# Eun0/XMC-GAN

Hardware: AMD Instinct MI355X
Metric: images/sec per G+D step (higher is better)
Workload: dtype bf16; 1 GPU; 256x256 COCO-shaped synthetic batch, 256 images per GPU, one full G+D iteration (D step + G step + Adam x2), df_gan_damsm_nomagp.yml; per_gpu_batch=256, global_batch=256, image_size=256, cfg=df_gan_damsm_nomagp.yml, parallelism=dp1, hipgraph=True, losses_finite=True, workload_name=headline

## Files before the change

include/xmc_gan_hip.h:

```cpp
#ifndef XMC_GAN_HIP_H
#define XMC_GAN_HIP_H

#include <stdint.h>

#ifdef __cplusplus
extern "C" {
#endif

#define XMC_ABI_VERSION 12

enum { XMC_BF16 = 0, XMC_F32 = 1 };
enum { XMC_HALF_IS_BF16 = 0, XMC_HALF_IS_F16 = 1 };
enum { XMC_ACT_NONE = 0, XMC_ACT_LRELU = 1, XMC_ACT_TANH = 2, XMC_ACT_RELU = 3 };
enum { XMC_EINVAL = -1, XMC_EALIGN = -2, XMC_ESHAPE = -3 };

#define XMC_MAX_TAPS 16
#define XMC_MAX_CLASSES 4

typedef struct XmcConvDesc {
    const void* src;
    const void* wpk;
    void* dst;
    const float* bias;
    const void* res;
    const float* alpha_dev;
    int32_t N, SH, SW, CS;
    int32_t DH, DW, CD;
    int32_t MH, MW;
    int32_t SA, DA;
    int32_t src_shift;
    int32_t ntaps, nclass;
    int32_t CDw;
    int32_t act;
    int32_t dtype;
    int32_t out_dtype;
    int8_t dh[XMC_MAX_CLASSES][XMC_MAX_TAPS];
    int8_t dw[XMC_MAX_CLASSES][XMC_MAX_TAPS];
    int8_t wi[XMC_MAX_CLASSES][XMC_MAX_TAPS];
    int8_t dph[XMC_MAX_CLASSES];
    int8_t dpw[XMC_MAX_CLASSES];
    const void* mask;
    float res_scale;
    int32_t res_mode;
    void* dst2;
    void* dst_pool;
    int32_t round_act;
    int32_t groups;
    int32_t post_act;
    float pool_scale;
    void* sign_bits;
    float* dot;
    const void* mask_bits;
    const void* sc_img;
    const void* sc_frag;
    const float* sc_bias;
    void* splitk_ws;
    int64_t splitk_ws_bytes;
    const void* wpk_lo;
} XmcConvDesc;

int xmc_abi_version(void);
int xmc_half_format(void);
const char* xmc_last_kernel(void);
int xmc_set_fixed_order(int on);
int xmc_set_prezeroed(int on);

int64_t xmc_conv_splitk_ws_bytes(const XmcConvDesc* d);

int xmc_conv_igemm(const XmcConvDesc* d, void* stream);

int xmc_conv_wgrad(const XmcConvDesc* d , float* dwp, void* stream);
#define XMC_BIAS_REPLICAS 16
int xmc_conv_wgrad_bias(const XmcConvDesc* d, float* dwp, float* dbias, void* stream);

int xmc_pack_weight(const float* w, void* wpk, int Co, int Ci, int KH, int KW, int rows_pad, int cols_pad,
                    int transpose , int dtype, const int32_t* row_perm , void* stream);
int xmc_pack_weight_grouped(const float* w, void* wpk, int Co, int Ci, int KH, int KW, int rows_pad, int cols_pad, int transpose,
                            int dtype, const int32_t* row_perm, int groups, void* stream);
int xmc_unpack_wgrad_grouped(const float* dwp, float* gw, int Co, int Ci, int KH, int KW, int rows_pad, int cols_pad,
                             const float* scale_dev, const int32_t* row_perm, int accumulate, int groups, void* stream);
#define XMC_PACK_MULTI_MAX 48
typedef struct XmcPackJob {
    const float* w;
    void* wpk;
    const int32_t* row_perm;
    int32_t Co, Ci, KHW, rows_pad, cols_pad, transpose, dtype, groups, upconv;
    int32_t lo;
} XmcPackJob;
int xmc_pack_weight_multi(const XmcPackJob* jobs , int njobs, void* stream);
int xmc_pack_weight_upconv(const float* w, void* wpk, int Co, int Ci, int rows_pad, int cols_pad, int transpose, int dtype,
                           void* stream);
int xmc_unpack_wgrad(const float* dwp, float* gw, int Co, int Ci, int KH, int KW, int rows_pad, int cols_pad,
                     const float* scale_dev, const int32_t* row_perm, int accumulate, void* stream);
int xmc_unpack_wgrad_bias(const float* dwp, float* gw, int Co, int Ci, int KH, int KW, int rows_pad, int cols_pad,
                          const float* scale_dev, const int32_t* row_perm, int accumulate,
                          const float* gb_replicas, float* gb, int CD, void* stream);
int xmc_unpack_wgrad_bias_dot(const float* dwp, float* gw, int Co, int Ci, int KH, int KW, int rows_pad, int cols_pad,
                              const float* scale_dev, const int32_t* row_perm, int accumulate,
                              const float* gb_replicas, float* gb, int CD, const float* bias_dot, float* dot, void* stream);

int xmc_nchw_to_nhwc8(const float* src , void* dst , int N, int C, int H, int W,
                      int dtype, void* stream);
int xmc_nhwc8_to_nchw(const void* src , float* dst , int N, int C, int H, int W,
                      int dtype, void* stream);

int xmc_lrelu(const void* x, void* y, int64_t n, float slope, int dtype, void* stream);
int xmc_lrelu_mask(const void* dy, const void* ref, void* dx, int64_t n, float slope, int dtype, void* stream);
int xmc_tanh(const void* x, void* y, int64_t n, int dtype, void* stream);
int xmc_signmask_apply(const void* dy, const void* bits, void* dx, int64_t n, float slope, int dtype, void* stream);
int xmc_conv_pw1x1_masked_src(const XmcConvDesc* d, const void* src_bits, void* src_masked, float slope, void* stream);
int xmc_conv_pw1x1_split(const XmcConvDesc* d, void* stream);
int xmc_conv_ptile_bits(const XmcConvDesc* d, void* stream);
int xmc_conv_ptile_scimg(const XmcConvDesc* d, void* stream);
int xmc_conv_wgrad_bits(const XmcConvDesc* d, float* dwp, void* stream);
int xmc_gtail_bwd(const XmcConvDesc* d, const void* img, float* dwp, float* dbias, int dw_rows, int grid_cap, void* stream);
int xmc_gentry_fwd(const void* x, const float* g0, const float* b0, const float* g1, const float* b1, const void* wpk, const float* bias,
                   void* h, void* sc, int N, int H, int W, int Cin, int Cout, int wrows, float slope, int dtype, int grid_cap, void* stream);
int xmc_gentry_bwd(const void* x, const void* dy, const void* dsc, const float* g0, const float* b0, const float* g1, const float* b1,
                   const void* wpk_t, void* dx, void* dx_pool, float* dg0, float* db0, float* dg1, float* db1, int N, int H, int W,
                   int Cin, int Cout, int wrows, float slope, int dtype, int grid_cap, void* stream);
int xmc_tanh_bwd(const void* dy, const void* y, void* dx, int64_t n, int dtype, void* stream);
int xmc_axpby(const void* a, const void* b, const float* alpha_dev, void* y, int64_t n, int dtype, void* stream);
int xmc_axpby_up(const void* a, const void* b, const float* alpha_dev, void* y, int N, int H, int W, int C, int dtype, void* stream);
int xmc_axpby_up_lrelu(const void* a, const void* b, const float* alpha_dev, void* y, int N, int H, int W, int C, int dtype, void* stream);
int xmc_scale(const void* x, const float* alpha_dev, void* y, int64_t n, int dtype, void* stream);
int xmc_dot(const void* a, const void* b, float* out, int64_t n, int dtype, void* stream);
enum { XMC_GP_BIAS = 1, XMC_GP_RELU = 2, XMC_GP_MASK = 4, XMC_GP_ATOMIC = 8 };
typedef struct XmcGemmProblem {
    const float* A;
    const float* B;
    const float* bias;
    const float* mask;
    float* C;
    float* rowsum;
    int32_t M, N, K;
    int32_t sa_i, sa_r, sb_j, sb_r;
    int32_t flags;
    int32_t tile0;
    int32_t reserved;
} XmcGemmProblem;
int xmc_gemm_group(const XmcGemmProblem* problems, int nproblems, void* stream);
int xmc_embedding_gather(const int64_t* ids, const float* table, float* out, int64_t n_tokens, int dim, int64_t vocab, void* stream);
int xmc_gru_bidir(const float* xproj, const float* w_hh, const float* b_hn, const int32_t* lens, float* words, float* sent, int B, int T,
                  int H, void* stream);
int xmc_lstm_bidir(const float* xproj, const float* w_hh, const int32_t* lens, float* words, float* sent, int B, int T, int H,
                   void* stream);
int xmc_roberta_embed_ln(const int64_t* ids, const int32_t* lens, const float* word, const float* pos, const float* type0,
                         const float* gamma, const float* beta, float* out, void* out16, int B, int T, int H, int64_t vocab, int npos,
                         int pad_idx, float eps, void* stream);
int xmc_add_layernorm(const float* x, const float* bias, const float* res, const float* gamma, const float* beta, float* out, void* out16,
                      int64_t rows, int H, float eps, void* stream);
int xmc_attention_short(const float* qkv, const int32_t* lens, void* out, int B, int T, int heads, int head_dim, int out_dtype,
                        void* stream);
int xmc_bias_gelu(const float* x, const float* bias, void* out, int64_t rows, int F, int out_dtype, void* stream);
int xmc_sbert_pool(const float* hidden, const int32_t* lens, float* words, float* sent, uint8_t* mask, int B, int T, int H, int L,
                   int normalize, void* stream);
int xmc_spectral_sigma(const float* W, float* u, float* v, float* scratch, float* sig, float* w_eff, int R, int C, int training,
                       float eps, void* stream);
int xmc_spectral_bwd(const float* g, const float* W, const float* u, const float* v, const float* sig, float* dot, float* dW,
                     int R, int C, void* stream);
int xmc_scale_mask_dot(const void* dy, const void* ref, const float* alpha_dev, void* g, float* dot, int64_t n, int dtype, void* stream);
int xmc_axpby_bwd(const void* dy, const void* b, const float* alpha_dev, void* db, void* da, float* dot,
                  int N, int H, int W, int C, int up, const void* ymask , int dtype, void* stream);
int xmc_colsum(const void* x, float* out, int64_t rows, int C, int dtype, void* stream);
int xmc_avgpool2(const void* x, void* y, int N, int H, int W, int C, int dtype, void* stream);
int xmc_upsample2(const void* x, void* y, int N, int H, int W, int C, float scale, int dtype, void* stream);
int xmc_sumpool2(const void* x, void* y, int N, int H, int W, int C, float scale, int dtype, void* stream);
int xmc_global_avgpool(const void* x, void* y, int N, int HW, int C, int dtype, int out_dtype, void* stream);
int xmc_global_avgpool_bwd(const void* dy, void* dx, int N, int HW, int C, int dtype, int in_dtype, void* stream);

int xmc_affine2_lrelu_fwd(const void* x, const float* g0, const float* b0, const float* g1, const float* b1,
                          void* y, int N, int HW, int C, int dtype, void* stream);
int xmc_affine2_lrelu_bwd(const void* x, const void* dy, const float* g0, const float* b0, const float* g1,
                          const float* b1, void* dx, float* dg0, float* db0, float* dg1, float* db1,
                          int N, int HW, int C, int dtype, void* stream);

int xmc_affine2_act_fwd(const void* x, const float* g0, const float* b0, const float* g1, const float* b1,
                        void* y, int N, int HW, int C, float slope, int dtype, void* stream);
int xmc_affine2_act_bwd(const void* x, const void* dy, const float* g0, const float* b0, const float* g1,
                        const float* b1, void* dx, float* dg0, float* db0, float* dg1, float* db1,
                        int N, int HW, int C, float slope, int dtype, void* stream);
int xmc_affine2_act_bwd_acc(const void* x, const void* dy, const float* g0, const float* b0, const float* g1,
                            const float* b1, void* dx, float* dg0, float* db0, float* dg1, float* db1, const void* dx_in,
                            int N, int HW, int C, float slope, int dtype, void* stream);
int xmc_affine2_act_bwd_dot(const void* x, const void* dy, const float* g0, const float* b0, const float* g1,
                            const float* b1, void* dx, float* dg0, float* db0, float* dg1, float* db1, const void* dx_in,
                            const float* alpha_dev, float* dot, int N, int HW, int C, float slope, int dtype, void* stream);
int xmc_affine2_act_bwd_dot_pool(const void* x, const void* dy, const float* g0, const float* b0, const float* g1,
                                 const float* b1, void* dx, float* dg0, float* db0, float* dg1, float* db1, const void* dx_in,
                                 const float* alpha_dev, float* dot, void* dx_pool, int N, int H, int W, int C, float slope,
                                 int dtype, void* stream);

int xmc_groupnorm_fwd(const void* x, const float* w, const float* b, void* y, float* stats, float* ws,
                      int N, int HW, int C, int G, float eps, float slope, int dtype, void* stream);
int xmc_groupnorm_bwd(const void* x, const void* dy, const float* w, const float* b, const float* stats, void* dx,
                      float* dw, float* db, float* ws, int N, int HW, int C, int G, float slope, int dtype, void* stream);
int64_t xmc_attn_pool_ws_floats(int N, int HW);
int xmc_attn_pool_fwd(const void* key, const float* q, const void* x, float* stats, float* ctx, float* ws, int N, int HW,
                      int ncon, int pk, int px, float scale, int dtype, void* stream);
int xmc_attn_pool_bwd(const void* key, const float* q, const void* x, const float* stats, const float* ctx, const float* dctx,
                      float* dq, void* dkey, void* dx, int N, int HW, int ncon, int pk, int px, float scale, int dtype, void* stream);
int xmc_attn_pool_bwd_acc(const void* key, const float* q, const void* x, const float* stats, const float* ctx, const float* dctx,
                          float* dq, void* dkey, void* dx, const void* dx_in, int N, int HW, int ncon, int pk, int px, float scale,
                          int dtype, void* stream);

int xmc_gvec_fwd(const float* xs, const float* xg, const float* W, const float* bias, float* y, int B, int G, int O, int Is, int Ig, void* stream);
int xmc_gvec_bwd(const float* xs, const float* xg, const float* W, const float* dy, float* dxs, float* dxg, float* dW, float* dbias,
                 int B, int G, int O, int Is, int Ig, void* stream);
int xmc_reasoner_fwd(const float* x, const float* We, const float* bn_w, const float* bn_b, float* run_mean, float* run_var, int training,
                     float momentum, float eps, float* y, float* pre, float* stat, int B, void* stream);
int xmc_reasoner_bwd(const float* x, const float* We, const float* bn_w, const float* bn_b, const float* pre, const float* stat, int batch_stats,
                     const float* dy, float* dx, float* dWe, float* dbn_w, float* dbn_b, int B, void* stream);
int xmc_word_ctx_fwd(const float* st, const float* w, const unsigned char* pad, float* ctx, float* prob, int B, int T, void* stream);
int xmc_word_ctx_bwd(const float* st, const float* w, const float* prob, const float* dctx, float* dst, float* dw, int B, int T, void* stream);
int xmc_word_keys_fwd(const float* kraw, const float* gnw, const float* gnb, float eps, float* kh, float* stat, int B, int T, void* stream);
int xmc_word_keys_bwd(const float* kraw, const float* gnw, const float* gnb, const float* stat, const float* dkh, float* dkraw, float* dgnw,
                      float* dgnb, int B, int T, void* stream);
int xmc_word_pool_fwd(const void* qmap, const float* kh, const unsigned char* pad, float* ctx, int N, int HW, int ncon, int pk, int T,
                      int dtype, void* stream);
int xmc_word_pool_bwd(const void* qmap, const float* kh, const unsigned char* pad, const float* dctx, void* dq, float* dkh, int N, int HW,
                      int ncon, int pk, int T, int dtype, void* stream);

int64_t xmc_contrastive_ws_bytes(int n, int D);
int xmc_contrastive_fwd(const float* A, const float* B, const float* labels, const float* inv_num_pos,
                        int n, int D, float* loss, void* ws, void* stream);
int xmc_contrastive_bwd(const float* A, const float* B, const float* labels, const float* inv_num_pos,
                        int n, int D, const float* dloss_dev, void* ws, float* dA, float* dB, void* stream);

int xmc_cosine_scores(const float* A, const float* B, int n, int D, float* S, void* ws, void* stream);

int xmc_hinge_fwd(const void* x, int stride, float sign, float* out, int64_t n, int dtype, void* stream);
int xmc_hinge_bwd(const void* x, int stride, float sign, const float* dloss_dev, void* dx, int64_t n, int dtype,
                  void* stream);

int xmc_cast(const void* x, void* y, int64_t n, int src_dtype, int dst_dtype, void* stream);

typedef struct XmcAdamEntry {
    float* param;
    const float* grad;
    float* m;
    float* v;
    int32_t* step;
    int64_t n;
} XmcAdamEntry;
int xmc_adam_chunk_elems(void);
int xmc_adam_step(const XmcAdamEntry* table_dev, int ntensors, const int32_t* chunks_dev, int nchunks,
                  float lr, float beta1, float beta2, float eps, float grad_scale, void* stream);
enum { XMC_ADAM_CHECK = 1, XMC_ADAM_UPDATE = 2, XMC_ADAM_RESCALE = 4 };
int xmc_adam_step_scaled(const XmcAdamEntry* table_dev, int ntensors, const int32_t* chunks_dev, int nchunks,
                         float lr, float beta1, float beta2, float eps, float* scale_dev, int32_t* flags_dev,
                         int mode, float growth, float backoff, int interval, void* stream);

typedef struct XmcEmaEntry {
    float* shadow;
    const float* param;
    int64_t n;
} XmcEmaEntry;
int xmc_ema_step(const XmcEmaEntry* table_dev, int ntensors, const int32_t* chunks_dev, int nchunks, float decay, int start,
                 int32_t* num_updates_dev, const int32_t* skip_flag_dev, int bump, void* stream);
int xmc_adam_ema_step(const XmcAdamEntry* table_dev, const XmcEmaEntry* ema_table_dev, int ntensors, const int32_t* chunks_dev,
                      int nchunks, float lr, float beta1, float beta2, float eps, float grad_scale, float decay, int start,
                      int32_t* num_updates_dev, int bump, void* stream);
int xmc_adam_ema_step_scaled(const XmcAdamEntry* table_dev, const XmcEmaEntry* ema_table_dev, int ntensors,
                             const int32_t* chunks_dev, int nchunks, float lr, float beta1, float beta2, float eps,
                             float* scale_dev, int32_t* flags_dev, int mode, float growth, float backoff, int interval,
                             float decay, int start, int32_t* num_updates_dev, int bump, void* stream);

int xmc_rows_sumsq(const float* x, float* ss, int B, int64_t cols, void* stream);
int xmc_gp_finish(const float* ss, int B, float* gp, float* coef, float inv_s2, void* stream);
int xmc_rows_scale(const float* x, const float* coef, const float* g, float* y, int B, int64_t cols, void* stream);

int xmc_concept_query_fwd(const float* sent, const float* Wq, const float* gnw, const float* gnb, float* q, float* qraw,
                          int B, int E, float eps, void* stream);
int xmc_concept_query_bwd(const float* sent, const float* Wq, const float* gnw, const float* qraw, const float* dq, float* dsent,
                          float* dWq, float* dgnw, float* dgnb, float* scratch, int B, int E, float eps, void* stream);
int xmc_concept_query_fwd_multi(const float* sent, const float* const* Wq, const float* const* gnw, const float* const* gnb, int S, float* q,
                                float* qraw, int B, int E, float eps, void* stream);
int xmc_concept_query_bwd_multi(const float* sent, const float* const* Wq, const float* const* gnw, int S, const float* qraw, const float* dq,
                                float* dsent, float* dWq, float* dgn, float* scratch, int B, int E, float eps, void* stream);
int xmc_concept_gquery_fwd(const float* q0, const float* Wq, const float* gnw, const float* gnb, float* q, float* qraw, int B,
                           float eps, void* stream);
int xmc_concept_gquery_bwd(const float* q0, const float* Wq, const float* gnw, const float* qraw, const float* dq, float* dq0,
                           float* dWq, float* dgnw, float* dgnb, int B, float eps, void* stream);
int xmc_concept_head_fwd(const float* ctx, const float* sent, const float* const* params, float* gamma, float* beta, float* hid,
                         int B, int E, void* stream);
int xmc_concept_head_fwd_pre(const float* ctx, const float* sent, const float* const* params, const float* a_pre, float* gamma, float* beta,
                             float* hid, int B, int E, void* stream);
int xmc_concept_head_bwd(const float* ctx, const float* sent, const float* hid, const float* const* params, const float* dgamma,
                         const float* dbeta, float* dctx, float* dsent, float* const* grads, float* scratch, int B, int E,
                         void* stream);
int xmc_concept_head_bwd_pre(const float* ctx, const float* sent, const float* hid, const float* const* params, const float* dgamma,
                             const float* dbeta, float* dctx, float* dsent, float* const* grads, float* scratch, int B, int E, void* stream);
int xmc_concept_outer_multi(const float* D, const float* X, const float* const* W, float* const* dW, int nW, int Rp, float* dX, int B, int C,
                            int ldw, void* stream);

int xmc_dstem_compose(const float* wi, const float* bi, const float* w0, const float* ws, const float* bs, float* W, float* bias, float* D,
                      float* DB, void* stream);
int xmc_dstem_compose_bwd(const float* wi, const float* bi, const float* w0, const float* ws, const float* dW, const float* dbias,
                          const float* dD, const float* dDB, float* dwi, float* dbi, float* dw0, float* dws, float* dbs, void* stream);
int xmc_dstem_pack(const float* wsets, void* wfrag, void* stream);
int xmc_dstem_pack_sc(const float* wsets, void* sc_frag, void* stream);
int xmc_dstem_fwd(const void* img, const void* wfrag, const float* bias, void* h1, void* sc, int N, int H, int W, float slope, void* stream);
int xmc_dstem_wgrad(const void* img, const void* dh1, const void* dsc, float* dw, float* dbias, int N, int H, int W, int skip_border,
                    void* stream);
int xmc_dstem_border_fwd(const void* img, const float* w, const float* bias, const float* D, const float* DB, void* frag_scratch ,
                         void* h1, int N, int H, int W, float slope, void* stream);
int xmc_dstem_border_wgrad(const void* img, const void* dh1, float* dD, float* dDB, int N, int H, int W, void* stream);
int xmc_dstem_dgrad(const void* dh1, const void* dsc, const float* wsets, const float* D, void* frag_scratch, void* dimg, int N, int H, int W,
                    void* stream);

#define XMC_DIFFAUG_PARTS 64
int xmc_diffaug_sums(const void* x, const float* params, float* parts, int N, int H, int W, int C, int cut, int transposed, int dtype,
                     void* stream);
int xmc_diffaug_apply(const void* x, const float* params, const float* parts, void* y, int N, int H, int W, int C, int cut, int transposed,
                      int linear_only, int dtype, void* stream);

int xmc_image_to_u8(const void* x, uint8_t* y, int N, int H, int W, int dtype, void* stream);
int xmc_image_minmax(const void* x, float* parts, int N, int H, int W, int dtype, void* stream);
int xmc_image_grid_u8(const void* x, const float* parts, uint8_t* grid, int N, int H, int W, int nrow, int padding, int dtype, void* stream);

int xmc_fid_resize_u8(const uint8_t* src, float* dst, int N, int H, int W, int OH, int OW, void* stream);
#define XMC_POOL_MAX 0
#define XMC_POOL_AVG_VALID 1
#define XMC_POOL_AVG_PAD 2
int xmc_pool3x3(const float* x, float* y, int N, int H, int W, int C, int mode, int stride, void* stream);
int xmc_resize_bilinear_f32(const float* src, float* dst, int N, int H, int W, int OH, int OW, void* stream);
int xmc_fid_moments(const float* x, double* sum, double* outer, int B, int D, void* stream);

int xmc_rprecision(const float* img, const float* txt, const int32_t* cand, int32_t* rank, float* score, int N, int M, int K, int D, void* stream);

int xmc_crop_flip_normalize(const uint8_t* pool, int64_t pool_bytes, const int64_t* offsets, const int32_t* hw, int N, const int32_t* params,
                            const float* table, float* out, int B, int S, void* stream);

int xmc_caption_gather(const float* sent_tab, const float* tok_tab, int64_t tok_rows, const int64_t* tok_offsets, const int32_t* lens, int N,
                       const int32_t* rows, int B, int E, int T, float* words, float* sent, uint8_t* mask, void* stream);

int xmc_manifold_slices(int Nq, int Nc, int slices);
int xmc_row_sqnorm(const float* x, float* n2, int N, int D, void* stream);
int xmc_knn_radius2(const float* x, const float* n2, float* r2, float* ws, int64_t ws_bytes, int N, int D, int k, int slices, void* stream);
int xmc_manifold_count(const float* a, const float* na2, const float* b, const float* nb2, const float* rb2, int32_t* count, float* near2,
                       void* ws, int64_t ws_bytes, int Na, int Nb, int D, int slices, void* stream);

int xmc_poly_mmd_tiles(int m);
int xmc_poly_mmd_sums(const float* real, const float* fake, const int32_t* idx_real, const int32_t* idx_fake, double* out, double* ws,
                      int64_t ws_bytes, int Nr, int Nf, int D, int S, int m, void* stream);
int64_t xmc_inception_score_ws_bytes(int N, int C, int splits);
int xmc_inception_score(const float* logits, int64_t ld, double* H, double* P, double* ws, int64_t ws_bytes, int N, int C, int splits,
                        void* stream);

#ifdef __cplusplus
}
#endif
#endif
```

xmc-gan_amd/csrc/adam.hip:

```cpp
#include "common.h"

namespace {
constexpr int NT = 256;
constexpr int CHUNK = NT * 4 * 4;

__global__ void adam_check_kernel(const XmcAdamEntry* __restrict__ tab, const int2* __restrict__ chunks, int* __restrict__ si) {
    const int2 c = chunks[blockIdx.x];
    const XmcAdamEntry e = tab[c.x];
    const int64_t base = (int64_t)c.y * CHUNK;
    const int64_t lim = e.n - base < CHUNK ? e.n - base : CHUNK;
    const float* g = e.grad + base;
    bool bad = false;
    if ((e.n & 3) == 0) {
        for (int i = threadIdx.x * 4; i < lim; i += NT * 4) {
            const f32x4 G = *reinterpret_cast<const f32x4*>(g + i);
            bad |= !(fabsf(G[0]) < INFINITY) | !(fabsf(G[1]) < INFINITY) | !(fabsf(G[2]) < INFINITY) | !(fabsf(G[3]) < INFINITY);
        }
    } else {
        for (int i = threadIdx.x; i < lim; i += NT) bad |= !(fabsf(g[i]) < INFINITY);
    }
    if (__builtin_amdgcn_ballot_w64(bad) != 0 && (threadIdx.x & 63) == 0) atomicOr(si, 1);
}
__global__ void scaler_update_kernel(float* __restrict__ sf, int* __restrict__ si, float growth, float backoff, int interval) {
    if (threadIdx.x != 0 || blockIdx.x != 0) return;
    float sc = sf[0];
    const int bad = si[0];
    if (bad) {
        sc = fmaxf(sc * backoff, 1.f);
        si[1] = 0;
        si[3] += 1;
    } else if (++si[1] >= interval) {
        sc = fminf(sc * growth, 16777216.f);
        si[1] = 0;
    }
    sf[0] = sc;
    sf[1] = 1.f / sc;
    si[2] = bad;
    si[0] = 0;
}

__global__ void adam_kernel(const XmcAdamEntry* __restrict__ tab, const int2* __restrict__ chunks,
                            float lr, float b1, float b2, float eps, float gs, const float* __restrict__ sf,
                            const int* __restrict__ si) {
    if (si && *si) return;
    if (sf) gs *= sf[1];
    const int2 c = chunks[blockIdx.x];
    const XmcAdamEntry e = tab[c.x];
    const int t = *e.step + 1;
    const float bc1 = 1.f - powf(b1, (float)t), bc2s = sqrtf(1.f - powf(b2, (float)t));
    const float step_size = lr / bc1;
    const int64_t base = (int64_t)c.y * CHUNK;
    const int64_t lim = e.n - base < CHUNK ? e.n - base : CHUNK;
    float* p = e.param + base; const float* g = e.grad + base; float* m = e.m + base; float* v = e.v + base;
    if ((e.n & 3) == 0) {
        for (int i = threadIdx.x * 4; i < lim; i += NT * 4) {
            f32x4 P = *reinterpret_cast<f32x4*>(p + i), G = *reinterpret_cast<const f32x4*>(g + i) * gs;
            f32x4 M = *reinterpret_cast<f32x4*>(m + i), V = *reinterpret_cast<f32x4*>(v + i);
#pragma unroll
            for (int k = 0; k < 4; ++k) {
                M[k] = b1 * M[k] + (1.f - b1) * G[k];
                V[k] = b2 * V[k] + (1.f - b2) * G[k] * G[k];
                P[k] -= step_size * M[k] / (sqrtf(V[k]) / bc2s + eps);
            }
            *reinterpret_cast<f32x4*>(p + i) = P; *reinterpret_cast<f32x4*>(m + i) = M; *reinterpret_cast<f32x4*>(v + i) = V;
        }
    } else {
        for (int i = threadIdx.x; i < lim; i += NT) {
            float G = g[i] * gs;
            float M = b1 * m[i] + (1.f - b1) * G;
            float V = b2 * v[i] + (1.f - b2) * G * G;
            p[i] -= step_size * M / (sqrtf(V) / bc2s + eps);
            m[i] = M; v[i] = V;
        }
    }
}
__global__ void adam_bump_kernel(const XmcAdamEntry* tab, int n, const int* __restrict__ si) {
    if (si && *si) return;
    int i = blockIdx.x * blockDim.x + threadIdx.x;
    if (i < n) *tab[i].step += 1;
}
}

extern "C" int xmc_adam_chunk_elems(void) { return CHUNK; }

extern "C" int xmc_adam_step(const XmcAdamEntry* table_dev, int ntensors, const int32_t* chunks_dev, int nchunks,
                             float lr, float beta1, float beta2, float eps, float grad_scale, void* stream) {
    if (!table_dev || !chunks_dev || ntensors < 1 || nchunks < 1) return XMC_EINVAL;
    hipStream_t st = reinterpret_cast<hipStream_t>(stream);
    hipLaunchKernelGGL(adam_kernel, dim3(nchunks), dim3(NT), 0, st, table_dev, reinterpret_cast<const int2*>(chunks_dev), lr, beta1, beta2, eps,
                       grad_scale, (const float*)nullptr, (const int*)nullptr);
    hipLaunchKernelGGL(adam_bump_kernel, dim3((ntensors + NT - 1) / NT), dim3(NT), 0, st, table_dev, ntensors, (const int*)nullptr);
    XMC_LAUNCH_CHECK();
    return 0;
}

extern "C" int xmc_adam_step_scaled(const XmcAdamEntry* table_dev, int ntensors, const int32_t* chunks_dev, int nchunks,
                                    float lr, float beta1, float beta2, float eps, float* scale_dev, int32_t* flags_dev,
                                    int mode, float growth, float backoff, int interval, void* stream) {
    if (!table_dev || !chunks_dev || ntensors < 1 || nchunks < 1 || !scale_dev || !flags_dev || interval < 1 || (mode & 7) == 0) return XMC_EINVAL;
    hipStream_t st = reinterpret_cast<hipStream_t>(stream);
    const int2* ch = reinterpret_cast<const int2*>(chunks_dev);
    if (mode & XMC_ADAM_CHECK) hipLaunchKernelGGL(adam_check_kernel, dim3(nchunks), dim3(NT), 0, st, table_dev, ch, flags_dev);
    if (mode & XMC_ADAM_UPDATE) {
        hipLaunchKernelGGL(adam_kernel, dim3(nchunks), dim3(NT), 0, st, table_dev, ch, lr, beta1, beta2, eps, 1.f, (const float*)scale_dev,
                           (const int*)flags_dev);
        hipLaunchKernelGGL(adam_bump_kernel, dim3((ntensors + NT - 1) / NT), dim3(NT), 0, st, table_dev, ntensors, (const int*)flags_dev);
    }
    if (mode & XMC_ADAM_RESCALE) hipLaunchKernelGGL(scaler_update_kernel, dim3(1), dim3(64), 0, st, scale_dev, flags_dev, growth, backoff, interval);
    XMC_LAUNCH_CHECK();
    return 0;
}

namespace {
__device__ __forceinline__ bool aligned16(const void* a) { return (reinterpret_cast<uintptr_t>(a) & 15) == 0; }
__device__ __forceinline__ float ema_elem(float e, float p, float w, bool copy) { return copy ? p : __builtin_fmaf(w, p - e, e); }

__global__ void ema_kernel(const XmcEmaEntry* __restrict__ tab, const int2* __restrict__ chunks, float decay, int start,
                           const int* __restrict__ nupd, const int* __restrict__ si) {
    if (si && *si) return;
    const int2 c = chunks[blockIdx.x];
    const XmcEmaEntry t = tab[c.x];
    const bool copy = *nupd < start;
    const float w = 1.f - decay;
    const int64_t base = (int64_t)c.y * CHUNK;
    const int lim = (int)(t.n - base < CHUNK ? t.n - base : CHUNK);
    float* e = t.shadow + base; const float* p = t.param + base;
    int body = 0;
    if (aligned16(e) && aligned16(p)) {
        body = lim & ~3;
        for (int i = threadIdx.x * 4; i < body; i += NT * 4) {
            f32x4 E = *reinterpret_cast<f32x4*>(e + i);
            const f32x4 P = *reinterpret_cast<const f32x4*>(p + i);
#pragma unroll
            for (int k = 0; k < 4; ++k) E[k] = ema_elem(E[k], P[k], w, copy);
            *reinterpret_cast<f32x4*>(e + i) = E;
        }
    }
    for (int i = body + threadIdx.x; i < lim; i += NT) e[i] = ema_elem(e[i], p[i], w, copy);
}

template <bool FMA>
__device__ __forceinline__ float adam_elem(float P, float G, float& M, float& V, float b1, float b2, float step_size, float bc2s,
                                           float eps) {
#pragma clang fp contract(off)
    const float t = (1.f - b1) * G, u = ((1.f - b2) * G) * G;
    M = FMA ? __builtin_fmaf(b1, M, t) : b1 * M + t;
    V = FMA ? __builtin_fmaf(b2, V, u) : b2 * V + u;
    return P - (step_size * M) / (sqrtf(V) / bc2s + eps);
}

template <bool FMA>
__device__ __forceinline__ void adam_ema_chunk(float* p, const float* g, float* m, float* v, float* sh, int lim, float gs, float b1,
                                               float b2, float step_size, float bc2s, float eps, float w, bool copy) {
    int body = 0;
    if (aligned16(p) && aligned16(g) && aligned16(m) && aligned16(v) && aligned16(sh)) {
        body = lim & ~3;
        for (int i = threadIdx.x * 4; i < body; i += NT * 4) {
            f32x4 P = *reinterpret_cast<f32x4*>(p + i), G = *reinterpret_cast<const f32x4*>(g + i);
            f32x4 M = *reinterpret_cast<f32x4*>(m + i), V = *reinterpret_cast<f32x4*>(v + i);
#pragma unroll
            for (int k = 0; k < 4; ++k) {
                float Mk = M[k], Vk = V[k];
                P[k] = adam_elem<FMA>(P[k], G[k] * gs, Mk, Vk, b1, b2, step_size, bc2s, eps);
                M[k] = Mk; V[k] = Vk;
            }
            *reinterpret_cast<f32x4*>(p + i) = P; *reinterpret_cast<f32x4*>(m + i) = M; *reinterpret_cast<f32x4*>(v + i) = V;
            if (sh) {
                f32x4 E = *reinterpret_cast<f32x4*>(sh + i);
#pragma unroll
                for (int k = 0; k < 4; ++k) E[k] = ema_elem(E[k], P[k], w, copy);
                *reinterpret_cast<f32x4*>(sh + i) = E;
            }
        }
    }
    for (int i = body + threadIdx.x; i < lim; i += NT) {
        float M = m[i], V = v[i];
        const float P = adam_elem<FMA>(p[i], g[i] * gs, M, V, b1, b2, step_size, bc2s, eps);
        p[i] = P; m[i] = M; v[i] = V;
        if (sh) sh[i] = ema_elem(sh[i], P, w, copy);
    }
}

__global__ void adam_ema_kernel(const XmcAdamEntry* __restrict__ tab, const XmcEmaEntry* __restrict__ ema,
                                const int2* __restrict__ chunks, float lr, float b1, float b2, float eps, float gs,
                                const float* __restrict__ sf, const int* __restrict__ si, float decay, int start,
                                const int* __restrict__ nupd) {
    if (si && *si) return;
    if (sf) gs *= sf[1];
    const int2 c = chunks[blockIdx.x];
    const XmcAdamEntry t = tab[c.x];
    const int step = *t.step + 1;
    const float bc1 = 1.f - powf(b1, (float)step), bc2s = sqrtf(1.f - powf(b2, (float)step));
    const float step_size = lr / bc1;
    const bool copy = *nupd < start;
    const float w = 1.f - decay;
    const int64_t base = (int64_t)c.y * CHUNK;
    const int lim = (int)(t.n - base < CHUNK ? t.n - base : CHUNK);
    float* sh = ema[c.x].shadow;
    if (sh) sh += base;
    if ((t.n & 3) == 0) adam_ema_chunk<true>(t.param + base, t.grad + base, t.m + base, t.v + base, sh, lim, gs, b1, b2, step_size, bc2s, eps, w, copy);
    else adam_ema_chunk<false>(t.param + base, t.grad + base, t.m + base, t.v + base, sh, lim, gs, b1, b2, step_size, bc2s, eps, w, copy);
}

__global__ void ema_bump_kernel(const XmcAdamEntry* tab, int n, const int* __restrict__ si, int* nupd, int bump) {
    if (si && *si) return;
    const int i = blockIdx.x * blockDim.x + threadIdx.x;
    if (tab && i < n) *tab[i].step += 1;
    if (bump && i == 0) *nupd += 1;
}

bool ema_args_ok(float decay, int start, const int32_t* nupd) { return nupd && decay >= 0.f && decay < 1.f && start >= 0; }
}

extern "C" int xmc_ema_step(const XmcEmaEntry* table_dev, int ntensors, const int32_t* chunks_dev, int nchunks, float decay,
                            int start, int32_t* num_updates_dev, const int32_t* skip_flag_dev, int bump, void* stream) {
    if (!table_dev || !chunks_dev || ntensors < 1 || nchunks < 1 || !ema_args_ok(decay, start, num_updates_dev)) return XMC_EINVAL;
    hipStream_t st = reinterpret_cast<hipStream_t>(stream);
    hipLaunchKernelGGL(ema_kernel, dim3(nchunks), dim3(NT), 0, st, table_dev, reinterpret_cast<const int2*>(chunks_dev), decay, start,
                       (const int*)num_updates_dev, (const int*)skip_flag_dev);
    if (bump)
        hipLaunchKernelGGL(ema_bump_kernel, dim3(1), dim3(64), 0, st, (const XmcAdamEntry*)nullptr, 0, (const int*)skip_flag_dev,
                           (int*)num_updates_dev, 1);
    XMC_LAUNCH_CHECK();
    return 0;
}

extern "C" int xmc_adam_ema_step(const XmcAdamEntry* table_dev, const XmcEmaEntry* ema_table_dev, int ntensors,
                                 const int32_t* chunks_dev, int nchunks, float lr, float beta1, float beta2, float eps,
                                 float grad_scale, float decay, int start, int32_t* num_updates_dev, int bump, void* stream) {
    if (!table_dev || !ema_table_dev || !chunks_dev || ntensors < 1 || nchunks < 1 || !ema_args_ok(decay, start, num_updates_dev))
        return XMC_EINVAL;
    hipStream_t st = reinterpret_cast<hipStream_t>(stream);
    hipLaunchKernelGGL(adam_ema_kernel, dim3(nchunks), dim3(NT), 0, st, table_dev, ema_table_dev, reinterpret_cast<const int2*>(chunks_dev),
                       lr, beta1, beta2, eps, grad_scale, (const float*)nullptr, (const int*)nullptr, decay, start,
                       (const int*)num_updates_dev);
    hipLaunchKernelGGL(ema_bump_kernel, dim3((ntensors + NT - 1) / NT), dim3(NT), 0, st, table_dev, ntensors, (const int*)nullptr,
                       (int*)num_updates_dev, bump);
    XMC_LAUNCH_CHECK();
    return 0;
}

extern "C" int xmc_adam_ema_step_scaled(const XmcAdamEntry* table_dev, const XmcEmaEntry* ema_table_dev, int ntensors,
                                        const int32_t* chunks_dev, int nchunks, float lr, float beta1, float beta2, float eps,
                                        float* scale_dev, int32_t* flags_dev, int mode, float growth, float backoff, int interval,
                                        float decay, int start, int32_t* num_updates_dev, int bump, void* stream) {
    if (!table_dev || !ema_table_dev || !chunks_dev || ntensors < 1 || nchunks < 1 || !scale_dev || !flags_dev || interval < 1 ||
        (mode & 7) == 0 || !ema_args_ok(decay, start, num_updates_dev))
        return XMC_EINVAL;
    hipStream_t st = reinterpret_cast<hipStream_t>(stream);
    const int2* ch = reinterpret_cast<const int2*>(chunks_dev);
    if (mode & XMC_ADAM_CHECK) hipLaunchKernelGGL(adam_check_kernel, dim3(nchunks), dim3(NT), 0, st, table_dev, ch, flags_dev);
    if (mode & XMC_ADAM_UPDATE) {
        hipLaunchKernelGGL(adam_ema_kernel, dim3(nchunks), dim3(NT), 0, st, table_dev, ema_table_dev, ch, lr, beta1, beta2, eps, 1.f,
                           (const float*)scale_dev, (const int*)flags_dev, decay, start, (const int*)num_updates_dev);
        hipLaunchKernelGGL(ema_bump_kernel, dim3((ntensors + NT - 1) / NT), dim3(NT), 0, st, table_dev, ntensors, (const int*)flags_dev,
                           (int*)num_updates_dev, bump);
    }
    if (mode & XMC_ADAM_RESCALE) hipLaunchKernelGGL(scaler_update_kernel, dim3(1), dim3(64), 0, st, scale_dev, flags_dev, growth, backoff, interval);
    XMC_LAUNCH_CHECK();
    return 0;
}
```

xmc-gan_amd/csrc/common.h:

```cpp
#pragma once
#include <hip/hip_runtime.h>
#include <stdint.h>

#include "xmc_gan_hip.h"

#ifdef XMC_H16_IS_F16
typedef _Float16 xmc_h16;
#define XMC_MFMA_16x16x32 __builtin_amdgcn_mfma_f32_16x16x32_f16
#define XMC_MFMA_32x32x16 __builtin_amdgcn_mfma_f32_32x32x16_f16
#define XMC_HALF_FORMAT 1
#else
typedef __bf16 xmc_h16;
#define XMC_MFMA_16x16x32 __builtin_amdgcn_mfma_f32_16x16x32_bf16
#define XMC_MFMA_32x32x16 __builtin_amdgcn_mfma_f32_32x32x16_bf16
#define XMC_HALF_FORMAT 0
#endif
typedef __attribute__((ext_vector_type(8))) xmc_h16 bf16x8;
typedef __attribute__((ext_vector_type(4))) xmc_h16 bf16x4;
typedef __attribute__((ext_vector_type(4))) float f32x4;
typedef __attribute__((__vector_size__(4 * sizeof(short)))) short xmc_s16x4;
typedef __attribute__((ext_vector_type(4))) uint32_t u32x4;
typedef __attribute__((ext_vector_type(2))) uint32_t u32x2;

#define XMC_LRELU 0.2f

static inline int xmc_esz(int dtype) { return dtype == XMC_BF16 ? 2 : 4; }

void xmc_note_kernel(const char* fmt, ...);
void xmc_note_generic_epi(const char* kernel, int mask);
bool xmc_debug_off(const char* token);
bool xmc_fixed_order();
hipError_t xmc_zero_acc(void* p, size_t bytes, hipStream_t st);

#define XMC_LAUNCH_CHECK()                                     \
    do {                                                       \
        hipError_t e__ = hipGetLastError();                    \
        if (e__ != hipSuccess) return -(1000 + (int)e__);      \
    } while (0)

#define XMC_MAX_DYN_LDS (160 * 1024 - 1024)
#define XMC_ALLOW_BIG_LDS(kernel)                                                                                              \
    do {                                                                                                                       \
        static bool once__ = false;                                                                                            \
        if (!once__) {                                                                                                         \
            (void)hipFuncSetAttribute(reinterpret_cast<const void*>(&kernel), hipFuncAttributeMaxDynamicSharedMemorySize,      \
                                      XMC_MAX_DYN_LDS);                                                                        \
            (void)hipGetLastError();                                                                                           \
            once__ = true;                                                                                                     \
        }                                                                                                                      \
    } while (0)

__device__ __forceinline__ bf16x4 xmc_ds_read_tr16(const void* p) {
    return __builtin_bit_cast(bf16x4, __builtin_amdgcn_ds_read_tr16_b64_v4i16((__attribute__((address_space(3))) xmc_s16x4*)(p)));
}

__device__ __forceinline__ float xmc_pin_f32(float v) {
    asm("" : "+v"(v));
    return v;
}
__device__ __forceinline__ float lrelu_f(float v) { return v > 0.f ? v : XMC_LRELU * v; }
__device__ __forceinline__ float tanh_fast(float v) {
    const float e = __builtin_amdgcn_exp2f(v * 2.8853900817779268f);
    return 1.f - 2.f * __builtin_amdgcn_rcpf(e + 1.f);
}
__device__ __forceinline__ float lrelu_slope(float ref) { return ref > 0.f ? 1.f : XMC_LRELU; }
__device__ __forceinline__ float tanh_bwd_f(float dy, float y) { return xmc_pin_f32(dy * (1.f - y * y)); }
__device__ __forceinline__ float affine2_fwd_f(float x, float g0, float b0, float g1, float b1, float slope, bool two) {
    float u = __builtin_fmaf(x, g0, b0);
    u = u > 0.f ? u : slope * u;
    const float t = __builtin_fmaf(u, g1, b1);
    return xmc_pin_f32(two ? (t > 0.f ? t : slope * t) : u);
}
template <int DT>
__device__ __forceinline__ void affine2_bwd_unit(float (&xv)[8], const float (&dv)[8], const float (&o)[8], bool has_in, bool two, float slope,
                                                 float al, float* dacc, const float (&G0)[8], const float (&B0)[8], const float (&G1)[8],
                                                 const float (&B1)[8], float (&sg0)[8], float (&sb0)[8], float (&sg1)[8], float (&sb1)[8]) {
#pragma unroll
    for (int k = 0; k < 8; ++k) {
        const float u = __builtin_fmaf(xv[k], G0[k], B0[k]);
        const float a1 = u > 0.f ? u : slope * u;
        const float v = __builtin_fmaf(a1, G1[k], B1[k]);
        if (dacc) {
            const float y2 = two ? (v > 0.f ? v : slope * v) : a1;
            *dacc += dv[k] * (DT == XMC_BF16 ? (float)(xmc_h16)y2 : y2);
        }
        const float dvk = dv[k] * al;
        const float dvv = two ? dvk * (v > 0.f ? 1.f : slope) : dvk;
        sg1[k] += dvv * a1; sb1[k] += dvv;
        const float du = dvv * G1[k] * (u > 0.f ? 1.f : slope);
        sg0[k] += du * xv[k]; sb0[k] += du;
        xv[k] = xmc_pin_f32(du * G0[k]);
    }
    if (has_in) {
#pragma unroll
        for (int k = 0; k < 8; ++k) xv[k] += o[k];
    }
}
__device__ __forceinline__ u32x4 xmc_apply_sign_bits(u32x4 v, unsigned b) {
    bf16x8 h = __builtin_bit_cast(bf16x8, v);
#pragma unroll
    for (int k = 0; k < 8; ++k) {
        const float f = (float)h[k];
        h[k] = (xmc_h16)(((b >> k) & 1u) ? f : XMC_LRELU * f);
    }
    return __builtin_bit_cast(u32x4, h);
}

template <int DT> struct Vec8;
template <> struct Vec8<XMC_BF16> {
    static constexpr int BYTES = 16;
    __device__ static __forceinline__ void load(const void* p, size_t idx8, float (&v)[8]) {
        bf16x8 t = reinterpret_cast<const bf16x8*>(p)[idx8];
#pragma unroll
        for (int i = 0; i < 8; ++i) v[i] = (float)t[i];
    }
    __device__ static __forceinline__ void store(void* p, size_t idx8, const float (&v)[8]) {
        bf16x8 t;
#pragma unroll
        for (int i = 0; i < 8; ++i) t[i] = (xmc_h16)v[i];
        reinterpret_cast<bf16x8*>(p)[idx8] = t;
    }
};
template <> struct Vec8<XMC_F32> {
    static constexpr int BYTES = 32;
    __device__ static __forceinline__ void load(const void* p, size_t idx8, float (&v)[8]) {
        const f32x4* q = reinterpret_cast<const f32x4*>(p) + idx8 * 2;
        f32x4 a = q[0], b = q[1];
#pragma unroll
        for (int i = 0; i < 4; ++i) { v[i] = a[i]; v[4 + i] = b[i]; }
    }
    __device__ static __forceinline__ void store(void* p, size_t idx8, const float (&v)[8]) {
        f32x4* q = reinterpret_cast<f32x4*>(p) + idx8 * 2;
        f32x4 a, b;
#pragma unroll
        for (int i = 0; i < 4; ++i) { a[i] = v[i]; b[i] = v[4 + i]; }
        q[0] = a; q[1] = b;
    }
};

struct XcdWalk { int first, step, end; };
__device__ __forceinline__ XcdWalk xmc_xcd_walk(int ntiles) {
    const int G = (int)gridDim.x, b = (int)blockIdx.x;
#ifdef XMC_XCD_HELPER_OFF
    return XcdWalk{b, G, ntiles};
#endif
    if ((G & 7) != 0 || G < 16) return XcdWalk{b, G, ntiles};
    const int T8 = (ntiles + 7) >> 3, base = (b & 7) * T8;
    return XcdWalk{base + (b >> 3), G >> 3, base + T8 < ntiles ? base + T8 : ntiles};
}
static inline int xmc_ab_grid(int g) {
    static const bool off = xmc_debug_off("no_xcd_map");
    return (off && g >= 16 && (g & 7) == 0) ? g - 1 : g;
}

__device__ __forceinline__ float xmc_xor1(float v) {
    return __builtin_bit_cast(float, __builtin_amdgcn_mov_dpp(__builtin_bit_cast(int, v), 0xB1, 0xF, 0xF, true));
}
__device__ __forceinline__ float xmc_xor2(float v) {
    return __builtin_bit_cast(float, __builtin_amdgcn_mov_dpp(__builtin_bit_cast(int, v), 0x4E, 0xF, 0xF, true));
}
__device__ __forceinline__ float wave_sum(float v) {
#pragma unroll
    for (int o = 32; o > 0; o >>= 1) v += __shfl_xor(v, o, 64);
    return v;
}
__device__ __forceinline__ float wave_max(float v) {
#pragma unroll
    for (int o = 32; o > 0; o >>= 1) v = fmaxf(v, __shfl_xor(v, o, 64));
    return v;
}

template <int ODT>
__device__ __forceinline__ void epilogue_tail(const XmcConvDesc& d, size_t idx8, size_t ridx8, float (&v)[8], float alpha, float* dacc = nullptr) {
    if (d.sign_bits) {
        unsigned b = 0;
#pragma unroll
        for (int k = 0; k < 8; ++k) b |= (v[k] > 0.f ? 1u : 0u) << k;
        reinterpret_cast<unsigned char*>(d.sign_bits)[idx8] = (unsigned char)b;
    }
    if (d.dst2) Vec8<ODT>::store(d.dst2, idx8, v);
    if (ODT == XMC_BF16 && (d.dst2 || d.round_act)) {
#pragma unroll
        for (int k = 0; k < 8; ++k) v[k] = (float)(xmc_h16)v[k];
    }
    float mk[8];
    if (d.mask) {
        Vec8<ODT>::load(d.mask, idx8, mk);
        if (d.dot && dacc) {
#pragma unroll
            for (int k = 0; k < 8; ++k) *dacc += v[k] * mk[k];
        }
    }
    if (d.alpha_dev) {
#pragma unroll
        for (int k = 0; k < 8; ++k) v[k] *= alpha;
    }
    if (d.mask) {
#pragma unroll
        for (int k = 0; k < 8; ++k) v[k] *= lrelu_slope(mk[k]);
    }
    if (d.res) {
        const float rs = d.res_scale == 0.f ? 1.f : d.res_scale;
        float rr[8];
        Vec8<ODT>::load(d.res, ridx8, rr);
#pragma unroll
        for (int k = 0; k < 8; ++k) v[k] += rs * rr[k];
    }
    if (d.post_act == XMC_ACT_LRELU) {
#pragma unroll
        for (int k = 0; k < 8; ++k) v[k] = lrelu_f(v[k]);
    }
    Vec8<ODT>::store(d.dst, idx8, v);
}

constexpr int kEpiBias = 1, kEpiLrelu = 2, kEpiRound = 4, kEpiDst2 = 8, kEpiAlpha = 16, kEpiMask = 32, kEpiRes = 64, kEpiPost = 128, kEpiPool = 256,
              kEpiSign = 512, kEpiDot = 1024, kEpiScImg = 2048;
constexpr int kEpiGSum = kEpiBias | kEpiRound | kEpiAlpha | kEpiRes;
constexpr int kEpiDKeep = kEpiLrelu | kEpiDst2 | kEpiAlpha | kEpiRes | kEpiPool;
constexpr int kEpiDFwd = kEpiLrelu | kEpiRound | kEpiAlpha | kEpiRes | kEpiPool;
constexpr int kEpiDLast = kEpiLrelu | kEpiDst2 | kEpiAlpha | kEpiRes;
constexpr int kEpiDLin = kEpiDst2 | kEpiAlpha | kEpiMask | kEpiRes;
constexpr int kEpiDKeepS = kEpiLrelu | kEpiRound | kEpiSign | kEpiAlpha | kEpiRes | kEpiPool;
constexpr int kEpiDLastS = kEpiLrelu | kEpiRound | kEpiSign | kEpiAlpha | kEpiRes;
constexpr int kEpiDgDot = kEpiMask | kEpiAlpha | kEpiDot;
static inline int xmc_epi_mask(const XmcConvDesc& d) {
    if ((d.act != XMC_ACT_NONE && d.act != XMC_ACT_LRELU) || d.out_dtype != XMC_BF16) return -1;
    return (d.bias ? kEpiBias : 0) | (d.act == XMC_ACT_LRELU ? kEpiLrelu : 0) | ((d.round_act && !d.dst2) ? kEpiRound : 0) | (d.dst2 ? kEpiDst2 : 0) |
           (d.alpha_dev ? kEpiAlpha : 0) | (d.mask ? kEpiMask : 0) | (d.res ? kEpiRes : 0) | (d.post_act == XMC_ACT_LRELU ? kEpiPost : 0) |
           (d.dst_pool ? kEpiPool : 0) | (d.sign_bits ? kEpiSign : 0) | (d.dot ? kEpiDot : 0) | (d.sc_img ? kEpiScImg : 0);
}

__device__ __forceinline__ size_t res_index8(const XmcConvDesc& d, size_t idx8, int n, int y, int x, int a, int b, int ch8) {
    if (d.res_mode == 0) return idx8;
    if (d.res_mode == 1) return ((size_t)(n * d.MH + a) * d.MW + b) * (d.CD >> 3) + ch8;
    return ((size_t)(n * (d.DH >> 1) + (y >> 1)) * (d.DW >> 1) + (x >> 1)) * (d.CD >> 3) + ch8;
}
```

xmc-gan_amd/csrc/pointwise.hip:

```cpp
#include "common.h"
#include <stdlib.h>
#include <string.h>
#include <cstdarg>
#include <cstdio>

namespace {

constexpr int NT = 256;
inline int nblocks(int64_t items, int per_block = NT, int cap = 256 * 16) {
    int64_t b = (items + per_block - 1) / per_block;
    if (b < 1) b = 1;
    return (int)(b > cap ? cap : b);
}

constexpr int UN = 4;
constexpr int STREAM_BLOCKS = 1024;
inline int sblocks(int64_t n8) { return nblocks((n8 + UN - 1) / UN, NT, STREAM_BLOCKS); }

template <int DT, class F>
__global__ void map1_kernel(const void* x, void* y, int64_t n8, F f) {
    for (int64_t base = (int64_t)blockIdx.x * (NT * UN); base < n8; base += (int64_t)gridDim.x * (NT * UN)) {
        float v[UN][8];
#pragma unroll
        for (int j = 0; j < UN; ++j) {
// ... 198 lines not shown
        int oh = (int)(p % OH);
        int n = (int)(p / OH);
        float acc[8] = {0, 0, 0, 0, 0, 0, 0, 0}, v[8];
#pragma unroll
        for (int dy = 0; dy < 2; ++dy)
#pragma unroll
            for (int dx = 0; dx < 2; ++dx) {
                Vec8<DT>::load(x, (((int64_t)n * H + 2 * oh + dy) * W + 2 * ow + dx) * C8 + cc, v);
#pragma unroll
                for (int k = 0; k < 8; ++k) acc[k] += v[k];
            }
#pragma unroll
        for (int k = 0; k < 8; ++k) acc[k] *= scale;
        Vec8<DT>::store(y, i, acc);
    }
}
template <int DT>
__global__ void up2_kernel(const void* x, void* y, int N, int H, int W, int C8, float scale) {
    const int OH = H * 2, OW = W * 2;
    const int64_t total = (int64_t)N * OH * OW * C8;
    for (int64_t i = blockIdx.x * (int64_t)blockDim.x + threadIdx.x; i < total; i += (int64_t)gridDim.x * blockDim.x) {
        int cc = (int)(i % C8);
        int64_t p = i / C8;
        int ow = (int)(p % OW); p /= OW;
        int oh = (int)(p % OH);
        int n = (int)(p / OH);
        float v[8];
        Vec8<DT>::load(x, (((int64_t)n * H + (oh >> 1)) * W + (ow >> 1)) * C8 + cc, v);
#pragma unroll
        for (int k = 0; k < 8; ++k) v[k] *= scale;
        Vec8<DT>::store(y, i, v);
    }
}
template <int DT, int OD>
__global__ void gap_kernel(const void* x, void* y, int N, int HW, int C8) {
    const int64_t total = (int64_t)N * C8;
    for (int64_t i = blockIdx.x * (int64_t)blockDim.x + threadIdx.x; i < total; i += (int64_t)gridDim.x * blockDim.x) {
        int cc = (int)(i % C8);
        int n = (int)(i / C8);
        float acc[8] = {0, 0, 0, 0, 0, 0, 0, 0}, v[8];
        for (int p = 0; p < HW; ++p) {
            Vec8<DT>::load(x, ((int64_t)n * HW + p) * C8 + cc, v);
#pragma unroll
            for (int k = 0; k < 8; ++k) acc[k] += v[k];
        }
        const float inv = 1.f / HW;
#pragma unroll
        for (int k = 0; k < 8; ++k) acc[k] *= inv;
        Vec8<OD>::store(y, i, acc);
    }
}
template <int DT>
__global__ void gap_big_kernel(const void* x, float* y, int HW, int C8, int pix_per_block) {
    const int n = blockIdx.y, groups = NT / C8;
    const int cc = threadIdx.x % C8, g = threadIdx.x / C8;
    float acc[8] = {0, 0, 0, 0, 0, 0, 0, 0}, v[8];
    const int p_end = min(HW, (int)(blockIdx.x + 1) * pix_per_block);
    if (g < groups)
        for (int p = blockIdx.x * pix_per_block + g; p < p_end; p += groups) {
            Vec8<DT>::load(x, ((size_t)n * HW + p) * C8 + cc, v);
#pragma unroll
            for (int k = 0; k < 8; ++k) acc[k] += v[k];
        }
    __shared__ float red[NT * 8];
#pragma unroll
    for (int k = 0; k < 8; ++k) red[threadIdx.x * 8 + k] = acc[k];
    __syncthreads();
    if (threadIdx.x < C8) {
        const float inv = 1.f / HW;
        float t[8] = {0, 0, 0, 0, 0, 0, 0, 0};
        for (int gg = 0; gg < groups; ++gg)
#pragma unroll
            for (int k = 0; k < 8; ++k) t[k] += red[(gg * C8 + threadIdx.x) * 8 + k];
#pragma unroll
        for (int k = 0; k < 8; ++k) atomicAdd(&y[((size_t)n * C8 + threadIdx.x) * 8 + k], t[k] * inv);
    }
}
template <int DT, int ID>
__global__ void gap_bwd_kernel(const void* dy, void* dx, int N, int HW, int C8) {
    const int64_t total = (int64_t)N * HW * C8;
    const float inv = 1.f / HW;
    for (int64_t i = blockIdx.x * (int64_t)blockDim.x + threadIdx.x; i < total; i += (int64_t)gridDim.x * blockDim.x) {
        int cc = (int)(i % C8);
        int n = (int)(i / ((int64_t)HW * C8));
        float v[8];
        Vec8<ID>::load(dy, (int64_t)n * C8 + cc, v);
#pragma unroll
        for (int k = 0; k < 8; ++k) v[k] *= inv;
        Vec8<DT>::store(dx, i, v);
    }
}

template <int DT>
__global__ void nchw_to_nhwc8_kernel(const float* src, void* dst, int N, int C, int HW) {
    const int64_t total = (int64_t)N * HW;
    for (int64_t i = blockIdx.x * (int64_t)blockDim.x + threadIdx.x; i < total; i += (int64_t)gridDim.x * blockDim.x) {
        int64_t n = i / HW, p = i - n * HW;
        float v[8] = {0, 0, 0, 0, 0, 0, 0, 0};
        for (int c = 0; c < C; ++c) v[c] = src[(n * C + c) * HW + p];
        Vec8<DT>::store(dst, i, v);
    }
}
template <int DT>
__global__ void nhwc8_to_nchw_kernel(const void* src, float* dst, int N, int C, int HW) {
    const int64_t total = (int64_t)N * HW;
    for (int64_t i = blockIdx.x * (int64_t)blockDim.x + threadIdx.x; i < total; i += (int64_t)gridDim.x * blockDim.x) {
        int64_t n = i / HW, p = i - n * HW;
        float v[8];
        Vec8<DT>::load(src, i, v);
        for (int c = 0; c < C; ++c) dst[(n * C + c) * HW + p] = v[c];
    }
}

template <int DT>
__global__ void affine2_fwd_kernel(const void* x, const float* g0, const float* b0, const float* g1, const float* b1,
                                   void* y, int HW, int C8, int pix_per_block, float slope) {
    const int n = blockIdx.y, groups = NT / C8;
    const int cc = threadIdx.x % C8, g = threadIdx.x / C8;
    if (g >= groups) return;
    float G0[8], B0[8], G1[8], B1[8];
    const size_t pb = ((size_t)n * C8 + cc) * 8;
    const bool two = g1 != nullptr;
#pragma unroll
    for (int k = 0; k < 8; ++k) { G0[k] = g0[pb + k]; B0[k] = b0[pb + k]; G1[k] = two ? g1[pb + k] : 1.f; B1[k] = two ? b1[pb + k] : 0.f; }
    const int p_end = min(HW, (int)(blockIdx.x + 1) * pix_per_block);
    for (int p = blockIdx.x * pix_per_block + g; p < p_end; p += groups) {
        float v[8];
        const size_t idx = ((size_t)n * HW + p) * C8 + cc;
        Vec8<DT>::load(x, idx, v);
#pragma unroll
        for (int k = 0; k < 8; ++k) v[k] = affine2_fwd_f(v[k], G0[k], B0[k], G1[k], B1[k], slope, two);
        Vec8<DT>::store(y, idx, v);
    }
}
template <int DT, bool POOL>
__global__ __launch_bounds__(NT, 2) void affine2_bwd_kernel(
                                   const void* x, const void* dy, const float* g0, const float* b0, const float* g1,
                                   const float* b1, void* dx, float* dg0, float* db0, float* dg1, float* db1,
                                   int HW, int C8, int pix_per_block, float slope, const void* dx_in,
                                   const float* alpha_dev, float* dot, void* dx_pool, int Wq) {
    const float al = alpha_dev ? *alpha_dev : 1.f;
    float dacc = 0.f;
    const int n = blockIdx.y, groups = NT / C8;
    const int cc = threadIdx.x % C8, g = threadIdx.x / C8;
    float G0[8], B0[8], G1[8], B1[8];
    float sg0[8], sb0[8], sg1[8], sb1[8];
    const size_t pb = ((size_t)n * C8 + cc) * 8;
    const bool two = g1 != nullptr;
#pragma unroll
    for (int k = 0; k < 8; ++k) {
        G0[k] = g0[pb + k]; B0[k] = b0[pb + k]; G1[k] = two ? g1[pb + k] : 1.f; B1[k] = two ? b1[pb + k] : 0.f;
        sg0[k] = sb0[k] = sg1[k] = sb1[k] = 0.f;
    }
    auto pixel = [&](size_t idx, float (&xv)[8], const float (&dv)[8], const float (&o)[8], float* acc8) {
        affine2_bwd_unit<DT>(xv, dv, o, dx_in != nullptr, two, slope, al, dot ? &dacc : nullptr, G0, B0, G1, B1, sg0, sb0, sg1, sb1);
        Vec8<DT>::store(dx, idx, xv);
        if (POOL) {
#pragma unroll
            for (int k = 0; k < 8; ++k) acc8[k] += DT == XMC_BF16 ? (float)(xmc_h16)xv[k] : xv[k];
        }
    };
    const int p_end = min(HW, (int)(blockIdx.x + 1) * pix_per_block);
    if (g < groups)
        for (int p = blockIdx.x * pix_per_block + g; p < p_end; p += POOL ? groups : 2 * groups) {
            if (!POOL) {
                float xv[8], dv[8], o[8], xw[8], dw[8], ow[8];
                const size_t idx = ((size_t)n * HW + p) * C8 + cc;
                const bool second = p + groups < p_end;
                const size_t idx2 = second ? idx + (size_t)groups * C8 : idx;
                Vec8<DT>::load(x, idx, xv);
                Vec8<DT>::load(x, idx2, xw);
                Vec8<DT>::load(dy, idx, dv);
                Vec8<DT>::load(dy, idx2, dw);
                if (dx_in) { Vec8<DT>::load(dx_in, idx, o); Vec8<DT>::load(dx_in, idx2, ow); }
                pixel(idx, xv, dv, o, nullptr);
                if (second) pixel(idx2, xw, dw, ow, nullptr);
            } else {
                const int W = 2 * Wq;
                const int qy = p / W, col = p - qy * W;
                const size_t i0 = (((size_t)n * (HW / W) * 2 + 2 * qy) * W + col) * C8 + cc, i1 = i0 + (size_t)W * C8;
                float x0[8], d0[8], o0[8], x1[8], d1[8], o1[8];
                Vec8<DT>::load(x, i0, x0); Vec8<DT>::load(x, i1, x1);
                Vec8<DT>::load(dy, i0, d0); Vec8<DT>::load(dy, i1, d1);
                if (dx_in) { Vec8<DT>::load(dx_in, i0, o0); Vec8<DT>::load(dx_in, i1, o1); }
                float acc8[8] = {0, 0, 0, 0, 0, 0, 0, 0};
                pixel(i0, x0, d0, o0, acc8);
                pixel(i1, x1, d1, o1, acc8);
#pragma unroll
                for (int k = 0; k < 8; ++k) acc8[k] += __shfl_xor(acc8[k], C8, 64);
                if ((col & 1) == 0) Vec8<DT>::store(dx_pool, (((size_t)n * (HW / W) + qy) * Wq + (col >> 1)) * C8 + cc, acc8);
            }
        }
    if (dot) {
        dacc = wave_sum(dacc);
        if ((threadIdx.x & 63) == 0) atomicAdd(dot, dacc);
    }
    __shared__ float red[NT * 8];
    float* outs[4] = {dg0, db0, dg1, db1};
    float* sums[4] = {sg0, sb0, sg1, sb1};
#pragma unroll
    for (int q = 0; q < 4; ++q) {
        if (!two && q >= 2) break;
        __syncthreads();
#pragma unroll
        for (int k = 0; k < 8; ++k) red[threadIdx.x * 8 + k] = sums[q][k];
        __syncthreads();
        if (threadIdx.x < C8) {
            float t[8] = {0, 0, 0, 0, 0, 0, 0, 0};
            for (int gg = 0; gg < groups; ++gg)
#pragma unroll
                for (int k = 0; k < 8; ++k) t[k] += red[(gg * C8 + threadIdx.x) * 8 + k];
#pragma unroll
            for (int k = 0; k < 8; ++k) atomicAdd(&outs[q][((size_t)n * C8 + threadIdx.x) * 8 + k], t[k]);
        }
    }
}

template <int DT>
__global__ void hinge_fwd_kernel(const void* x, int stride, float sign, float* out, int64_t n) {
    float s = 0.f;
    for (int64_t i = threadIdx.x; i < n; i += blockDim.x) {
        float v = DT == XMC_BF16 ? (float)reinterpret_cast<const xmc_h16*>(x)[i * stride] : reinterpret_cast<const float*>(x)[i * stride];
        s += fmaxf(1.f + sign * v, 0.f);
    }
    s = wave_sum(s);
    __shared__ float part[NT / 64];
    if ((threadIdx.x & 63) == 0) part[threadIdx.x >> 6] = s;
    __syncthreads();
    if (threadIdx.x == 0) {
        float t = 0.f;
        for (int w = 0; w < NT / 64; ++w) t += part[w];
        *out = t / (float)n;
    }
}
template <int DT>
__global__ void hinge_bwd_kernel(const void* x, int stride, float sign, const float* dloss, void* dx, int64_t n) {
    const float gscale = (*dloss) * sign / (float)n;
    for (int64_t i = blockIdx.x * (int64_t)blockDim.x + threadIdx.x; i < n; i += (int64_t)gridDim.x * blockDim.x) {
        float v = DT == XMC_BF16 ? (float)reinterpret_cast<const xmc_h16*>(x)[i * stride] : reinterpret_cast<const float*>(x)[i * stride];
        float gval = (1.f + sign * v) > 0.f ? gscale : 0.f;
        if (DT == XMC_BF16) reinterpret_cast<xmc_h16*>(dx)[i * stride] = (xmc_h16)gval;
        else reinterpret_cast<float*>(dx)[i * stride] = gval;
    }
}

__device__ __forceinline__ float pack_value(const float* __restrict__ w, int Co, int Ci, int KHW, int rows_pad, int cols_pad,
                                            int transpose, const int32_t* __restrict__ row_perm, int groups, int64_t i) {
    const int cog = Co / groups, cig = Ci / groups;
    int c = (int)(i % cols_pad);
    int64_t q = i / cols_pad;
    int r = (int)(q % rows_pad);
    int t = (int)(q / rows_pad);
    int co = transpose ? c : r, ci = transpose ? r : c;
    float v = 0.f;
    if (co < Co && ci < Ci) {
        int sco = row_perm ? row_perm[co] : co;
        if (groups == 1) v = w[((int64_t)sco * Ci + ci) * KHW + t];
        else if (sco / cog == ci / cig) v = w[((int64_t)sco * cig + ci % cig) * KHW + t];
    }
    return v;
}
__device__ __forceinline__ float pack_upconv_value(const float* __restrict__ w, int Co, int Ci, int rows_pad, int cols_pad,
                                                   int transpose, int64_t idx) {
    int c = (int)(idx % cols_pad);
    int64_t q = idx / cols_pad;
    int r = (int)(q % rows_pad);
    int sl = (int)(q / rows_pad);
    int cls = sl >> 2, t = sl & 3;
    int i = cls >> 1, j = cls & 1, th = t >> 1, tw = t & 1;
    int co = transpose ? c : r, ci = transpose ? r : c;
    float v = 0.f;
    if (co < Co && ci < Ci) {
        int kh0 = (i == 0) ? (th == 0 ? 0 : 1) : (th == 0 ? 0 : 2), kh1 = (i == 0) ? (th == 0 ? 0 : 2) : (th == 0 ? 1 : 2);
        int kw0 = (j == 0) ? (tw == 0 ? 0 : 1) : (tw == 0 ? 0 : 2), kw1 = (j == 0) ? (tw == 0 ? 0 : 2) : (tw == 0 ? 1 : 2);
        const float* wp = w + ((int64_t)co * Ci + ci) * 9;
        for (int kh = kh0; kh <= kh1; ++kh)
            for (int kw = kw0; kw <= kw1; ++kw) v += wp[kh * 3 + kw];
    }
    return v;
}
template <int DT>
__global__ void pack_weight_kernel(const float* w, void* wpk, int Co, int Ci, int KHW, int rows_pad, int cols_pad,
                                   int transpose, const int32_t* row_perm, int groups) {
    const int64_t total = (int64_t)KHW * rows_pad * cols_pad;
    for (int64_t i = blockIdx.x * (int64_t)blockDim.x + threadIdx.x; i < total; i += (int64_t)gridDim.x * blockDim.x) {
        const float v = pack_value(w, Co, Ci, KHW, rows_pad, cols_pad, transpose, row_perm, groups, i);
        if (DT == XMC_BF16) reinterpret_cast<xmc_h16*>(wpk)[i] = (xmc_h16)v;
        else reinterpret_cast<float*>(wpk)[i] = v;
    }
}
template <int DT>
__global__ void pack_upconv_kernel(const float* w, void* wpk, int Co, int Ci, int rows_pad, int cols_pad, int transpose) {
    const int64_t total = (int64_t)16 * rows_pad * cols_pad;
    for (int64_t idx = blockIdx.x * (int64_t)blockDim.x + threadIdx.x; idx < total; idx += (int64_t)gridDim.x * blockDim.x) {
        const float v = pack_upconv_value(w, Co, Ci, rows_pad, cols_pad, transpose, idx);
        if (DT == XMC_BF16) reinterpret_cast<xmc_h16*>(wpk)[idx] = (xmc_h16)v;
        else reinterpret_cast<float*>(wpk)[idx] = v;
    }
}
constexpr int PM_CHUNK = 2048;
struct PackJobs { XmcPackJob j[XMC_PACK_MULTI_MAX]; int32_t first[XMC_PACK_MULTI_MAX + 1]; int32_t njobs; };
template <int DT>
__device__ __forceinline__ void pack_store(void* p, int64_t i, float v, bool lo = false) {
    if (DT == XMC_BF16) reinterpret_cast<xmc_h16*>(p)[i] = lo ? (xmc_h16)(v - (float)(xmc_h16)v) : (xmc_h16)v;
    else reinterpret_cast<float*>(p)[i] = v;
}
template <int DT>
__device__ __forceinline__ void pack_position(const XmcPackJob& job, int pos) {
    const int c = pos % job.cols_pad, r = pos / job.cols_pad;
    const int co = job.transpose ? c : r, ci = job.transpose ? r : c;
    const int64_t plane = (int64_t)job.rows_pad * job.cols_pad;
    const bool in = co < job.Co && ci < job.Ci;
    if (job.upconv) {
        float w9[9];
#pragma unroll
        for (int t = 0; t < 9; ++t) w9[t] = in ? job.w[((int64_t)co * job.Ci + ci) * 9 + t] : 0.f;
#pragma unroll
        for (int sl = 0; sl < 16; ++sl) {
            const int i = sl >> 3, j = (sl >> 2) & 1, th = (sl >> 1) & 1, tw = sl & 1;
            const int kh0 = (i == 0) ? (th == 0 ? 0 : 1) : (th == 0 ? 0 : 2), kh1 = (i == 0) ? (th == 0 ? 0 : 2) : (th == 0 ? 1 : 2);
            const int kw0 = (j == 0) ? (tw == 0 ? 0 : 1) : (tw == 0 ? 0 : 2), kw1 = (j == 0) ? (tw == 0 ? 0 : 2) : (tw == 0 ? 1 : 2);
            float v = 0.f;
#pragma unroll
            for (int kh = 0; kh < 3; ++kh)
#pragma unroll
                for (int kw = 0; kw < 3; ++kw)
                    if (kh >= kh0 && kh <= kh1 && kw >= kw0 && kw <= kw1) v += w9[kh * 3 + kw];
            pack_store<DT>(job.wpk, sl * plane + pos, v);
        }
        return;
    }
    const int cog = job.Co / job.groups, cig = job.Ci / job.groups;
    const float* src = nullptr;
    if (in) {
        const int sco = job.row_perm ? job.row_perm[co] : co;
        if (job.groups == 1) src = job.w + ((int64_t)sco * job.Ci + ci) * job.KHW;
        else if (sco / cog == ci / cig) src = job.w + ((int64_t)sco * cig + ci % cig) * job.KHW;
    }
    for (int t = 0; t < job.KHW; ++t) pack_store<DT>(job.wpk, t * plane + pos, src ? src[t] : 0.f, job.lo != 0);
}
__global__ __launch_bounds__(256) void pack_multi_kernel(const PackJobs J) {
    int jb = 0;
    while (jb + 1 < J.njobs && (int)blockIdx.x >= J.first[jb + 1]) ++jb;
    const XmcPackJob& job = J.j[jb];
    const int total = job.rows_pad * job.cols_pad;
    const int p0 = ((int)blockIdx.x - J.first[jb]) * PM_CHUNK;
    const int p1 = p0 + PM_CHUNK < total ? p0 + PM_CHUNK : total;
    if (job.dtype == XMC_BF16) for (int pos = p0 + threadIdx.x; pos < p1; pos += 256) pack_position<XMC_BF16>(job, pos);
    else for (int pos = p0 + threadIdx.x; pos < p1; pos += 256) pack_position<XMC_F32>(job, pos);
}
template <int DT>
__global__ void axpby_up_kernel(const void* a, const void* b, const float* alpha, void* y, int N, int H, int W, int C8, int lrelu) {
    const float al = *alpha;
    const int OH = 2 * H, OW = 2 * W;
    const int64_t total = (int64_t)N * OH * OW * C8;
    for (int64_t idx = blockIdx.x * (int64_t)blockDim.x + threadIdx.x; idx < total; idx += (int64_t)gridDim.x * blockDim.x) {
        int cc = (int)(idx % C8);
        int64_t p = idx / C8;
        int ow = (int)(p % OW); p /= OW;
        int oh = (int)(p % OH);
        int n = (int)(p / OH);
        float u[8], v[8];
        Vec8<DT>::load(a, (((int64_t)n * H + (oh >> 1)) * W + (ow >> 1)) * C8 + cc, u);
        Vec8<DT>::load(b, idx, v);
#pragma unroll
        for (int k = 0; k < 8; ++k) u[k] += al * v[k];
        if (lrelu) {
#pragma unroll
            for (int k = 0; k < 8; ++k) u[k] = lrelu_f(u[k]);
        }
        Vec8<DT>::store(y, idx, u);
    }
}

template <int DT>
__global__ void axpby_bwd_kernel(const void* dy, const void* b, const float* alpha, void* db, void* da, float* dot,
                                 int N, int H, int W, int C8, int up, const void* ymask) {
    const float al = *alpha;
    float s = 0.f;
    const int64_t total = (int64_t)N * H * W * C8;
    for (int64_t idx = blockIdx.x * (int64_t)blockDim.x + threadIdx.x; idx < total; idx += (int64_t)gridDim.x * blockDim.x) {
        if (!up) {
            float u[8], v[8], o[8];
            Vec8<DT>::load(dy, idx, u);
            Vec8<DT>::load(b, idx, v);
            if (ymask) {
                float mk[8];
                Vec8<DT>::load(ymask, idx, mk);
#pragma unroll
                for (int k = 0; k < 8; ++k) u[k] *= lrelu_slope(mk[k]);
                Vec8<DT>::store(da, idx, u);
            }
#pragma unroll
            for (int k = 0; k < 8; ++k) { s += u[k] * v[k]; o[k] = al * u[k]; }
            if (db) Vec8<DT>::store(db, idx, o);
            continue;
        }
        const int cc = (int)(idx % C8);
        int64_t p = idx / C8;
        const int w = (int)(p % W); p /= W;
        const int h = (int)(p % H);
        const int n = (int)(p / H);
        float sum[8] = {0.f, 0.f, 0.f, 0.f, 0.f, 0.f, 0.f, 0.f};
#pragma unroll
        for (int i = 0; i < 2; ++i)
#pragma unroll
            for (int j = 0; j < 2; ++j) {
                const int64_t hi = ((((int64_t)n * 2 * H + 2 * h + i) * 2 * W) + 2 * w + j) * C8 + cc;
                float u[8], v[8], o[8];
                Vec8<DT>::load(dy, hi, u);
                Vec8<DT>::load(b, hi, v);
                if (ymask) {
                    float mk[8];
                    Vec8<DT>::load(ymask, hi, mk);
#pragma unroll
                    for (int k = 0; k < 8; ++k) u[k] *= lrelu_slope(mk[k]);
                }
#pragma unroll
                for (int k = 0; k < 8; ++k) { s += u[k] * v[k]; o[k] = al * u[k]; sum[k] += u[k]; }
                if (db) Vec8<DT>::store(db, hi, o);
            }
        Vec8<DT>::store(da, idx, sum);
    }
    s = wave_sum(s);
    __shared__ float part[NT / 64];
    if ((threadIdx.x & 63) == 0) part[threadIdx.x >> 6] = s;
    __syncthreads();
    if (threadIdx.x == 0) {
        float t = 0.f;
        for (int w_ = 0; w_ < NT / 64; ++w_) t += part[w_];
        atomicAdd(dot, t);
    }
}

__global__ void unpack_wgrad_kernel(const float* dwp, float* gw, int Co, int Ci, int KHW, int rows_pad, int cols_pad,
                                    const float* scale_dev, const int32_t* row_perm, int accumulate,
                                    const float* gb_rep, float* gb, int CDb, int groups,
                                    const float* bias_dot, float* dot) {
    const float scale = scale_dev ? *scale_dev : 1.f;
    const int cog = Co / groups, cig = Ci / groups;
    const int64_t total = (int64_t)Co * cig * KHW;
    if (gb_rep) {
        for (int c = blockIdx.x * blockDim.x + threadIdx.x; c < CDb; c += gridDim.x * blockDim.x) {
            float sacc = 0.f;
#pragma unroll
            for (int r = 0; r < XMC_BIAS_REPLICAS; ++r) sacc += gb_rep[r * CDb + c];
            gb[c] = scale * sacc;
            if (bias_dot && c < Co) atomicAdd(dot, bias_dot[c] * sacc);
        }
    }
    for (int64_t i = blockIdx.x * (int64_t)blockDim.x + threadIdx.x; i < total; i += (int64_t)gridDim.x * blockDim.x) {
        int t = (int)(i % KHW);
        int64_t q = i / KHW;
        int ci = (int)(q % cig);
        int r = (int)(q / cig);
        int dco = row_perm ? row_perm[r] : r;
        float v = scale * dwp[((int64_t)t * rows_pad + r) * cols_pad + (dco / cog) * cig + ci];
        int64_t o = ((int64_t)dco * cig + ci) * KHW + t;
        gw[o] = accumulate ? gw[o] + v : v;
    }
}

__global__ void rows_sumsq_kernel(const float* __restrict__ x, float* __restrict__ ss, int64_t cols4) {
    const f32x4* row = reinterpret_cast<const f32x4*>(x) + (int64_t)blockIdx.y * cols4;
    float s = 0.f;
    for (int64_t i = blockIdx.x * (int64_t)blockDim.x + threadIdx.x; i < cols4; i += (int64_t)gridDim.x * blockDim.x) {
        const f32x4 v = row[i];
        s += v[0] * v[0] + v[1] * v[1] + v[2] * v[2] + v[3] * v[3];
    }
    s = wave_sum(s);
    __shared__ float part[NT / 64];
    if ((threadIdx.x & 63) == 0) part[threadIdx.x >> 6] = s;
    __syncthreads();
    if (threadIdx.x == 0) {
        float t = 0.f;
        for (int w = 0; w < NT / 64; ++w) t += part[w];
        atomicAdd(&ss[blockIdx.y], t);
    }
}
__global__ void gp_finish_kernel(const float* __restrict__ ss, int B, float* __restrict__ gp, float* __restrict__ coef, float inv_s2) {
    float s = 0.f;
    for (int b = threadIdx.x; b < B; b += blockDim.x) {
        const float v = ss[b] * inv_s2;
        s += v * v * v;
        coef[b] = 6.f * v * v / (float)B * inv_s2;
    }
    s = wave_sum(s);
    __shared__ float part[NT / 64];
    if ((threadIdx.x & 63) == 0) part[threadIdx.x >> 6] = s;
    __syncthreads();
    if (threadIdx.x == 0) {
        float t = 0.f;
        for (int w = 0; w < NT / 64; ++w) t += part[w];
        *gp = t / (float)B;
    }
}
__global__ void rows_scale_kernel(const float* __restrict__ x, const float* __restrict__ coef, const float* __restrict__ g,
                                  float* __restrict__ y, int64_t cols4) {
    const float c = coef[blockIdx.y] * (*g);
    const f32x4* row = reinterpret_cast<const f32x4*>(x) + (int64_t)blockIdx.y * cols4;
    f32x4* out = reinterpret_cast<f32x4*>(y) + (int64_t)blockIdx.y * cols4;
    for (int64_t i = blockIdx.x * (int64_t)blockDim.x + threadIdx.x; i < cols4; i += (int64_t)gridDim.x * blockDim.x) {
        f32x4 v = row[i];
        v[0] *= c; v[1] *= c; v[2] *= c; v[3] *= c;
        out[i] = v;
    }
}

}

#define ST(s) reinterpret_cast<hipStream_t>(s)

extern "C" int xmc_abi_version(void) { return XMC_ABI_VERSION; }
extern "C" int xmc_half_format(void) { return XMC_HALF_FORMAT; }

static thread_local char g_last_kernel[96] = "";
void xmc_note_kernel(const char* fmt, ...) {
    va_list ap;
    va_start(ap, fmt);
    vsnprintf(g_last_kernel, sizeof g_last_kernel, fmt, ap);
    va_end(ap);
}
extern "C" const char* xmc_last_kernel(void) { return g_last_kernel; }

void xmc_note_generic_epi(const char* kernel, int mask) {
    static const bool on = xmc_debug_off("log_generic_epi");
    if (!on || mask < 0) return;
    static char seen[64][96];
    static int nseen = 0;
    char key[96];
    snprintf(key, sizeof key, "%s epi=%d", kernel, mask);
    for (int i = 0; i < nseen; ++i)
        if (!strcmp(seen[i], key)) return;
    if (nseen < 64) strcpy(seen[nseen++], key);
    fprintf(stderr, "[xmc] generic epilogue: %s (bias %d lrelu %d round %d dst2 %d alpha %d mask %d res %d post %d pool %d)\n", key, mask & 1, (mask >> 1) & 1,
            (mask >> 2) & 1, (mask >> 3) & 1, (mask >> 4) & 1, (mask >> 5) & 1, (mask >> 6) & 1, (mask >> 7) & 1, (mask >> 8) & 1);
}

static int g_fixed_order = 0;
extern "C" int xmc_set_fixed_order(int on) { const int was = g_fixed_order; g_fixed_order = on ? 1 : 0; return was; }
bool xmc_fixed_order() { return g_fixed_order != 0; }
static int g_prezeroed = 0;
extern "C" int xmc_set_prezeroed(int on) { const int was = g_prezeroed; g_prezeroed = on ? 1 : 0; return was; }
hipError_t xmc_zero_acc(void* p, size_t bytes, hipStream_t st) { return g_prezeroed ? hipSuccess : hipMemsetAsync(p, 0, bytes, st); }

bool xmc_debug_off(const char* token) {
    static const char* env = getenv("XMC_DEBUG_DISPATCH");
    if (!env || !*env) return false;
    const size_t n = strlen(token);
    for (const char* p = env; (p = strstr(p, token)) != nullptr; p += n)
        if ((p == env || p[-1] == ',') && (p[n] == 0 || p[n] == ',')) return true;
    return false;
}

extern "C" int xmc_lrelu(const void* x, void* y, int64_t n, float slope, int dtype, void* s) { return run_map1(x, y, n, dtype, ST(s), FLrelu{slope}); }
extern "C" int xmc_tanh(const void* x, void* y, int64_t n, int dtype, void* s) { return run_map1(x, y, n, dtype, ST(s), FTanh{}); }
extern "C" int xmc_lrelu_mask(const void* dy, const void* ref, void* dx, int64_t n, float slope, int dtype, void* s) {
    return run_map2(dy, ref, dx, n, dtype, ST(s), FLreluMask{slope});
}
extern "C" int xmc_signmask_apply(const void* dy, const void* bits, void* dx, int64_t n, float slope, int dtype, void* s) {
    if (!dy || !bits || !dx) return XMC_EINVAL;
    if (n % 8) return XMC_EALIGN;
    if (n == 0) return 0;
    const int64_t n8 = n / 8;
    if (dtype == XMC_BF16) hipLaunchKernelGGL((signmask_kernel<XMC_BF16>), dim3(sblocks(n8)), dim3(NT), 0, ST(s), dy, (const unsigned char*)bits, dx, n8, slope);
    else if (dtype == XMC_F32) hipLaunchKernelGGL((signmask_kernel<XMC_F32>), dim3(sblocks(n8)), dim3(NT), 0, ST(s), dy, (const unsigned char*)bits, dx, n8, slope);
    else return XMC_EINVAL;
    XMC_LAUNCH_CHECK();
    return 0;
}
extern "C" int xmc_tanh_bwd(const void* dy, const void* y, void* dx, int64_t n, int dtype, void* s) {
    return run_map2(dy, y, dx, n, dtype, ST(s), FTanhBwd{});
}
extern "C" int xmc_axpby(const void* a, const void* b, const float* alpha, void* y, int64_t n, int dtype, void* s) {
    if (!alpha) return XMC_EINVAL;
    return run_map2(a, b, y, n, dtype, ST(s), FAxpby{alpha});
}
extern "C" int xmc_scale(const void* x, const float* alpha, void* y, int64_t n, int dtype, void* s) {
    if (!alpha) return XMC_EINVAL;
    return run_map1(x, y, n, dtype, ST(s), FScale{alpha});
}
extern "C" int xmc_cast(const void* x, void* y, int64_t n, int src_dtype, int dst_dtype, void* s) {
    if (n % 8) return XMC_EALIGN;
    if (n == 0) return 0;
    int64_t n8 = n / 8;
    dim3 g(nblocks(n8)), b(NT);
    if (src_dtype == XMC_F32 && dst_dtype == XMC_BF16) hipLaunchKernelGGL((cast_kernel<XMC_F32, XMC_BF16>), g, b, 0, ST(s), x, y, n8);
    else if (src_dtype == XMC_BF16 && dst_dtype == XMC_F32) hipLaunchKernelGGL((cast_kernel<XMC_BF16, XMC_F32>), g, b, 0, ST(s), x, y, n8);
    else if (src_dtype == XMC_F32 && dst_dtype == XMC_F32) hipLaunchKernelGGL((cast_kernel<XMC_F32, XMC_F32>), g, b, 0, ST(s), x, y, n8);
    else if (src_dtype == XMC_BF16 && dst_dtype == XMC_BF16) hipLaunchKernelGGL((cast_kernel<XMC_BF16, XMC_BF16>), g, b, 0, ST(s), x, y, n8);
    else return XMC_EINVAL;
    XMC_LAUNCH_CHECK();
    return 0;
}
extern "C" int xmc_dot(const void* a, const void* b, float* out, int64_t n, int dtype, void* s) {
    if (n % 8) return XMC_EALIGN;
    int64_t n8 = n / 8;
    dim3 g(nblocks(n8, NT, 512)), blk(NT);
    if (dtype == XMC_BF16) hipLaunchKernelGGL((dot_kernel<XMC_BF16>), g, blk, 0, ST(s), a, b, out, n8);
    else if (dtype == XMC_F32) hipLaunchKernelGGL((dot_kernel<XMC_F32>), g, blk, 0, ST(s), a, b, out, n8);
    else return XMC_EINVAL;
    XMC_LAUNCH_CHECK();
    return 0;
}
extern "C" int xmc_scale_mask_dot(const void* dy, const void* ref, const float* alpha, void* g, float* dot, int64_t n, int dtype, void* s) {
    if (n % 8) return XMC_EALIGN;
    int64_t n8 = n / 8;
    dim3 grd(sblocks(n8)), blk(NT);
    if (dtype == XMC_BF16) hipLaunchKernelGGL((scale_mask_dot_kernel<XMC_BF16>), grd, blk, 0, ST(s), dy, ref, alpha, g, dot, n8);
    else if (dtype == XMC_F32) hipLaunchKernelGGL((scale_mask_dot_kernel<XMC_F32>), grd, blk, 0, ST(s), dy, ref, alpha, g, dot, n8);
    else return XMC_EINVAL;
    XMC_LAUNCH_CHECK();
    return 0;
}
extern "C" int xmc_colsum(const void* x, float* out, int64_t rows, int C, int dtype, void* s) {
    if (C % 8) return XMC_EALIGN;
    const int C8 = C / 8, groups = C8 >= NT ? 1 : NT / C8;
    dim3 g(nblocks(rows, groups * 8, 1024), (C8 + NT - 1) / NT), blk(NT);
    if (dtype == XMC_BF16) hipLaunchKernelGGL((colsum_kernel<XMC_BF16>), g, blk, 0, ST(s), x, out, rows, C8);
    else if (dtype == XMC_F32) hipLaunchKernelGGL((colsum_kernel<XMC_F32>), g, blk, 0, ST(s), x, out, rows, C8);
    else return XMC_EINVAL;
    XMC_LAUNCH_CHECK();
    return 0;
}
static int pool2(const void* x, void* y, int N, int H, int W, int C, float scale, int dtype, void* s) {
    if (C % 8 || H % 2 || W % 2) return XMC_EALIGN;
    int64_t total = (int64_t)N * (H / 2) * (W / 2) * (C / 8);
    dim3 g(nblocks(total)), blk(NT);
    if (dtype == XMC_BF16) hipLaunchKernelGGL((pool2_kernel<XMC_BF16>), g, blk, 0, ST(s), x, y, N, H, W, C / 8, scale);
    else if (dtype == XMC_F32) hipLaunchKernelGGL((pool2_kernel<XMC_F32>), g, blk, 0, ST(s), x, y, N, H, W, C / 8, scale);
    else return XMC_EINVAL;
    XMC_LAUNCH_CHECK();
// ... 298 lines not shown
```

xmc-gan_amd/lib.py:

```python
import ctypes as C
import os

HERE = os.path.dirname(os.path.abspath(__file__))
LIB_PATH = os.environ.get("XMC_LIB_PATH", os.path.join(HERE, "libxmc_gan_hip.so"))
LIB_PATH_F16 = os.environ.get("XMC_LIB_PATH_F16", os.path.join(HERE, "libxmc_gan_hip_f16.so"))
ABI_VERSION = 12

BF16, F32 = 0, 1
H16 = BF16
ACT_NONE, ACT_LRELU, ACT_TANH, ACT_RELU = 0, 1, 2, 3
MAX_TAPS, MAX_CLASSES = 16, 4
POOL_MAX, POOL_AVG_VALID, POOL_AVG_PAD = 0, 1, 2
DIFFAUG_PARTS = 64

vp, i32, i64, f32 = C.c_void_p, C.c_int32, C.c_int64, C.c_float


class ConvDesc(C.Structure):
    _fields_ = [("src", vp), ("wpk", vp), ("dst", vp), ("bias", vp), ("res", vp), ("alpha_dev", vp),
                ("N", i32), ("SH", i32), ("SW", i32), ("CS", i32),
                ("DH", i32), ("DW", i32), ("CD", i32),
                ("MH", i32), ("MW", i32), ("SA", i32), ("DA", i32), ("src_shift", i32),
                ("ntaps", i32), ("nclass", i32), ("CDw", i32), ("act", i32), ("dtype", i32), ("out_dtype", i32),
                ("dh", (C.c_int8 * MAX_TAPS) * MAX_CLASSES), ("dw", (C.c_int8 * MAX_TAPS) * MAX_CLASSES),
                ("wi", (C.c_int8 * MAX_TAPS) * MAX_CLASSES),
                ("dph", C.c_int8 * MAX_CLASSES), ("dpw", C.c_int8 * MAX_CLASSES),
                ("mask", vp), ("res_scale", f32), ("res_mode", i32), ("dst2", vp), ("dst_pool", vp), ("round_act", i32), ("groups", i32),
                ("post_act", i32), ("pool_scale", f32), ("sign_bits", vp), ("dot", vp), ("mask_bits", vp), ("sc_img", vp), ("sc_frag", vp), ("sc_bias", vp),
                ("splitk_ws", vp), ("splitk_ws_bytes", C.c_int64), ("wpk_lo", vp)]


GEMM_PROBLEM = [("A", "u8"), ("B", "u8"), ("bias", "u8"), ("mask", "u8"), ("C", "u8"), ("rowsum", "u8"),
                ("M", "i4"), ("N", "i4"), ("K", "i4"), ("sa_i", "i4"), ("sa_r", "i4"), ("sb_j", "i4"), ("sb_r", "i4"),
                ("flags", "i4"), ("tile0", "i4"), ("reserved", "i4")]
GP_BIAS, GP_RELU, GP_MASK, GP_ATOMIC = 1, 2, 4, 8


class PackJob(C.Structure):
    _fields_ = [("w", vp), ("wpk", vp), ("row_perm", vp), ("Co", i32), ("Ci", i32), ("KHW", i32), ("rows_pad", i32),
                ("cols_pad", i32), ("transpose", i32), ("dtype", i32), ("groups", i32), ("upconv", i32), ("lo", i32)]


class AdamEntry(C.Structure):
    _fields_ = [("param", vp), ("grad", vp), ("m", vp), ("v", vp), ("step", vp), ("n", i64)]


class EmaEntry(C.Structure):
    _fields_ = [("shadow", vp), ("param", vp), ("n", i64)]


_SIGS = {
    "xmc_abi_version": [],
    "xmc_half_format": [],
    "xmc_last_kernel": [],
    "xmc_set_fixed_order": [i32],
    "xmc_set_prezeroed": [i32],
    "xmc_conv_splitk_ws_bytes": [vp],
    "xmc_conv_igemm": [C.POINTER(ConvDesc), vp],
    "xmc_conv_wgrad": [C.POINTER(ConvDesc), vp, vp],
    "xmc_conv_wgrad_bias": [C.POINTER(ConvDesc), vp, vp, vp],
    "xmc_pack_weight": [vp, vp, i32, i32, i32, i32, i32, i32, i32, i32, vp, vp],
    "xmc_pack_weight_grouped": [vp, vp, i32, i32, i32, i32, i32, i32, i32, i32, vp, i32, vp],
    "xmc_pack_weight_upconv": [vp, vp, i32, i32, i32, i32, i32, i32, vp],
    "xmc_pack_weight_multi": [C.POINTER(PackJob), i32, vp],
    "xmc_axpby_up": [vp, vp, vp, vp, i32, i32, i32, i32, i32, vp],
    "xmc_unpack_wgrad": [vp, vp, i32, i32, i32, i32, i32, i32, vp, vp, i32, vp],
    "xmc_unpack_wgrad_grouped": [vp, vp, i32, i32, i32, i32, i32, i32, vp, vp, i32, i32, vp],
    "xmc_unpack_wgrad_bias": [vp, vp, i32, i32, i32, i32, i32, i32, vp, vp, i32, vp, vp, i32, vp],
    "xmc_unpack_wgrad_bias_dot": [vp, vp, i32, i32, i32, i32, i32, i32, vp, vp, i32, vp, vp, i32, vp, vp, vp],
    "xmc_nchw_to_nhwc8": [vp, vp, i32, i32, i32, i32, i32, vp],
    "xmc_nhwc8_to_nchw": [vp, vp, i32, i32, i32, i32, i32, vp],
    "xmc_lrelu": [vp, vp, i64, f32, i32, vp],
    "xmc_lrelu_mask": [vp, vp, vp, i64, f32, i32, vp],
    "xmc_tanh": [vp, vp, i64, i32, vp],
    "xmc_signmask_apply": [vp, vp, vp, i64, f32, i32, vp],
    "xmc_conv_pw1x1_masked_src": [C.POINTER(ConvDesc), vp, vp, f32, vp],
    "xmc_conv_pw1x1_split": [C.POINTER(ConvDesc), vp],
    "xmc_conv_ptile_bits": [C.POINTER(ConvDesc), vp],
    "xmc_conv_ptile_scimg": [C.POINTER(ConvDesc), vp],
    "xmc_conv_wgrad_bits": [C.POINTER(ConvDesc), vp, vp],
    "xmc_gtail_bwd": [C.POINTER(ConvDesc), vp, vp, vp, i32, i32, vp],
    "xmc_gentry_fwd": [vp, vp, vp, vp, vp, vp, vp, vp, vp, i32, i32, i32, i32, i32, i32, f32, i32, i32, vp],
    "xmc_gentry_bwd": [vp, vp, vp, vp, vp, vp, vp, vp, vp, vp, vp, vp, vp, vp, i32, i32, i32, i32, i32, i32, f32, i32, i32, vp],
    "xmc_tanh_bwd": [vp, vp, vp, i64, i32, vp],
    "xmc_axpby": [vp, vp, vp, vp, i64, i32, vp],
    "xmc_scale_mask_dot": [vp, vp, vp, vp, vp, i64, i32, vp],
    "xmc_axpby_bwd": [vp, vp, vp, vp, vp, vp, i32, i32, i32, i32, i32, vp, i32, vp],
    "xmc_axpby_up_lrelu": [vp, vp, vp, vp, i32, i32, i32, i32, i32, vp],
    "xmc_scale": [vp, vp, vp, i64, i32, vp],
    "xmc_dot": [vp, vp, vp, i64, i32, vp],
    "xmc_gemm_group": [vp, i32, vp],
    "xmc_embedding_gather": [vp, vp, vp, i64, i32, i64, vp],
    "xmc_lstm_bidir": [vp, vp, vp, vp, vp, i32, i32, i32, vp],
    "xmc_gru_bidir": [vp, vp, vp, vp, vp, vp, i32, i32, i32, vp],
    "xmc_roberta_embed_ln": [vp, vp, vp, vp, vp, vp, vp, vp, vp, i32, i32, i32, i64, i32, i32, f32, vp],
    "xmc_add_layernorm": [vp, vp, vp, vp, vp, vp, vp, i64, i32, f32, vp],
    "xmc_attention_short": [vp, vp, vp, i32, i32, i32, i32, i32, vp],
    "xmc_bias_gelu": [vp, vp, vp, i64, i32, i32, vp],
    "xmc_sbert_pool": [vp, vp, vp, vp, vp, i32, i32, i32, i32, i32, vp],
    "xmc_spectral_sigma": [vp, vp, vp, vp, vp, vp, i32, i32, i32, f32, vp],
    "xmc_spectral_bwd": [vp, vp, vp, vp, vp, vp, vp, i32, i32, vp],
    "xmc_colsum": [vp, vp, i64, i32, i32, vp],
    "xmc_avgpool2": [vp, vp, i32, i32, i32, i32, i32, vp],
    "xmc_upsample2": [vp, vp, i32, i32, i32, i32, f32, i32, vp],
    "xmc_sumpool2": [vp, vp, i32, i32, i32, i32, f32, i32, vp],
    "xmc_global_avgpool": [vp, vp, i32, i32, i32, i32, i32, vp],
    "xmc_global_avgpool_bwd": [vp, vp, i32, i32, i32, i32, i32, vp],
    "xmc_affine2_act_fwd": [vp, vp, vp, vp, vp, vp, i32, i32, i32, f32, i32, vp],
    "xmc_affine2_act_bwd": [vp, vp, vp, vp, vp, vp, vp, vp, vp, vp, vp, i32, i32, i32, f32, i32, vp],
    "xmc_affine2_act_bwd_acc": [vp, vp, vp, vp, vp, vp, vp, vp, vp, vp, vp, vp, i32, i32, i32, f32, i32, vp],
    "xmc_affine2_act_bwd_dot": [vp, vp, vp, vp, vp, vp, vp, vp, vp, vp, vp, vp, vp, vp, i32, i32, i32, f32, i32, vp],
    "xmc_affine2_act_bwd_dot_pool": [vp, vp, vp, vp, vp, vp, vp, vp, vp, vp, vp, vp, vp, vp, vp, i32, i32, i32, i32, f32, i32, vp],
    "xmc_affine2_lrelu_fwd": [vp, vp, vp, vp, vp, vp, i32, i32, i32, i32, vp],
    "xmc_affine2_lrelu_bwd": [vp, vp, vp, vp, vp, vp, vp, vp, vp, vp, vp, i32, i32, i32, i32, vp],
    "xmc_groupnorm_fwd": [vp, vp, vp, vp, vp, vp, i32, i32, i32, i32, f32, f32, i32, vp],
    "xmc_groupnorm_bwd": [vp, vp, vp, vp, vp, vp, vp, vp, vp, i32, i32, i32, i32, f32, i32, vp],
    "xmc_attn_pool_ws_floats": [i32, i32],
    "xmc_attn_pool_fwd": [vp, vp, vp, vp, vp, vp, i32, i32, i32, i32, i32, f32, i32, vp],
    "xmc_attn_pool_bwd": [vp, vp, vp, vp, vp, vp, vp, vp, vp, i32, i32, i32, i32, i32, f32, i32, vp],
    "xmc_attn_pool_bwd_acc": [vp, vp, vp, vp, vp, vp, vp, vp, vp, vp, i32, i32, i32, i32, i32, f32, i32, vp],
    "xmc_word_pool_fwd": [vp, vp, vp, vp, i32, i32, i32, i32, i32, i32, vp],
    "xmc_word_pool_bwd": [vp, vp, vp, vp, vp, vp, i32, i32, i32, i32, i32, i32, vp],
    "xmc_gvec_fwd": [vp, vp, vp, vp, vp, i32, i32, i32, i32, i32, vp],
    "xmc_gvec_bwd": [vp, vp, vp, vp, vp, vp, vp, vp, i32, i32, i32, i32, i32, vp],
    "xmc_reasoner_fwd": [vp, vp, vp, vp, vp, vp, i32, f32, f32, vp, vp, vp, i32, vp],
    "xmc_reasoner_bwd": [vp, vp, vp, vp, vp, vp, i32, vp, vp, vp, vp, vp, i32, vp],
    "xmc_word_ctx_fwd": [vp, vp, vp, vp, vp, i32, i32, vp],
    "xmc_word_ctx_bwd": [vp, vp, vp, vp, vp, vp, i32, i32, vp],
    "xmc_word_keys_fwd": [vp, vp, vp, f32, vp, vp, i32, i32, vp],
    "xmc_word_keys_bwd": [vp, vp, vp, vp, vp, vp, vp, vp, i32, i32, vp],
    "xmc_contrastive_ws_bytes": [i32, i32],
    "xmc_contrastive_fwd": [vp, vp, vp, vp, i32, i32, vp, vp, vp],
    "xmc_contrastive_bwd": [vp, vp, vp, vp, i32, i32, vp, vp, vp, vp, vp],
    "xmc_cosine_scores": [vp, vp, i32, i32, vp, vp, vp],
    "xmc_hinge_fwd": [vp, i32, f32, vp, i64, i32, vp],
    "xmc_hinge_bwd": [vp, i32, f32, vp, vp, i64, i32, vp],
    "xmc_cast": [vp, vp, i64, i32, i32, vp],
    "xmc_concept_query_fwd": [vp, vp, vp, vp, vp, vp, i32, i32, f32, vp],
    "xmc_concept_query_bwd": [vp, vp, vp, vp, vp, vp, vp, vp, vp, vp, i32, i32, f32, vp],
    "xmc_concept_query_fwd_multi": [vp, vp, vp, vp, i32, vp, vp, i32, i32, f32, vp],
    "xmc_concept_query_bwd_multi": [vp, vp, vp, i32, vp, vp, vp, vp, vp, vp, i32, i32, f32, vp],
    "xmc_concept_gquery_fwd": [vp, vp, vp, vp, vp, vp, i32, f32, vp],
    "xmc_concept_gquery_bwd": [vp, vp, vp, vp, vp, vp, vp, vp, vp, i32, f32, vp],
    "xmc_concept_head_fwd": [vp, vp, vp, vp, vp, vp, i32, i32, vp],
    "xmc_concept_head_fwd_pre": [vp, vp, vp, vp, vp, vp, vp, i32, i32, vp],
    "xmc_concept_head_bwd_pre": [vp, vp, vp, vp, vp, vp, vp, vp, vp, vp, i32, i32, vp],
    "xmc_concept_outer_multi": [vp, vp, vp, vp, i32, i32, vp, i32, i32, i32, vp],
    "xmc_concept_head_bwd": [vp, vp, vp, vp, vp, vp, vp, vp, vp, vp, i32, i32, vp],
    "xmc_rows_sumsq": [vp, vp, i32, i64, vp],
    "xmc_gp_finish": [vp, i32, vp, vp, f32, vp],
    "xmc_rows_scale": [vp, vp, vp, vp, i32, i64, vp],
    "xmc_adam_chunk_elems": [],
    "xmc_adam_step": [vp, i32, vp, i32, f32, f32, f32, f32, f32, vp],
    "xmc_adam_step_scaled": [vp, i32, vp, i32, f32, f32, f32, f32, vp, vp, i32, f32, f32, i32, vp],
    "xmc_ema_step": [vp, i32, vp, i32, f32, i32, vp, vp, i32, vp],
    "xmc_adam_ema_step": [vp, vp, i32, vp, i32, f32, f32, f32, f32, f32, f32, i32, vp, i32, vp],
    "xmc_adam_ema_step_scaled": [vp, vp, i32, vp, i32, f32, f32, f32, f32, vp, vp, i32, f32, f32, i32, f32, i32, vp, i32, vp],
    "xmc_dstem_compose": [vp, vp, vp, vp, vp, vp, vp, vp, vp, vp],
    "xmc_dstem_compose_bwd": [vp, vp, vp, vp, vp, vp, vp, vp, vp, vp, vp, vp, vp, vp],
    "xmc_dstem_pack": [vp, vp, vp],
    "xmc_dstem_pack_sc": [vp, vp, vp],
    "xmc_dstem_fwd": [vp, vp, vp, vp, vp, i32, i32, i32, f32, vp],
    "xmc_dstem_wgrad": [vp, vp, vp, vp, vp, i32, i32, i32, i32, vp],
    "xmc_dstem_border_fwd": [vp, vp, vp, vp, vp, vp, vp, i32, i32, i32, f32, vp],
    "xmc_dstem_border_wgrad": [vp, vp, vp, vp, i32, i32, i32, vp],
    "xmc_dstem_dgrad": [vp, vp, vp, vp, vp, vp, i32, i32, i32, vp],
    "xmc_diffaug_sums": [vp, vp, vp, i32, i32, i32, i32, i32, i32, i32, vp],
    "xmc_diffaug_apply": [vp, vp, vp, vp, i32, i32, i32, i32, i32, i32, i32, i32, vp],
    "xmc_image_to_u8": [vp, vp, i32, i32, i32, i32, vp],
    "xmc_image_minmax": [vp, vp, i32, i32, i32, i32, vp],
    "xmc_image_grid_u8": [vp, vp, vp, i32, i32, i32, i32, i32, i32, vp],
    "xmc_fid_resize_u8": [vp, vp, i32, i32, i32, i32, i32, vp],
    "xmc_pool3x3": [vp, vp, i32, i32, i32, i32, i32, i32, vp],
    "xmc_fid_moments": [vp, vp, vp, i32, i32, vp],
    "xmc_resize_bilinear_f32": [vp, vp, i32, i32, i32, i32, i32, vp],
    "xmc_rprecision": [vp, vp, vp, vp, vp, i32, i32, i32, i32, vp],
    "xmc_crop_flip_normalize": [vp, i64, vp, vp, i32, vp, vp, vp, i32, i32, vp],
    "xmc_caption_gather": [vp, vp, i64, vp, vp, i32, vp, i32, i32, i32, vp, vp, vp, vp],
    "xmc_manifold_slices": [i32, i32, i32],
    "xmc_row_sqnorm": [vp, vp, i32, i32, vp],
    "xmc_knn_radius2": [vp, vp, vp, vp, i64, i32, i32, i32, i32, vp],
    "xmc_manifold_count": [vp, vp, vp, vp, vp, vp, vp, vp, i64, i32, i32, i32, i32, vp],
    "xmc_poly_mmd_tiles": [i32],
    "xmc_poly_mmd_sums": [vp, vp, vp, vp, vp, vp, i64, i32, i32, i32, i32, i32, vp],
    "xmc_inception_score_ws_bytes": [i32, i32, i32],
    "xmc_inception_score": [vp, i64, vp, vp, vp, i64, i32, i32, i32, vp],
}
_RESTYPE = {"xmc_contrastive_ws_bytes": i64, "xmc_conv_splitk_ws_bytes": i64, "xmc_attn_pool_ws_floats": i64, "xmc_last_kernel": C.c_char_p,
            "xmc_inception_score_ws_bytes": i64}
EXPORTS = tuple(_SIGS)

_libs = {}
_variant = "bf16"


class XmcHipError(RuntimeError):
    pass


def use_variant(v):
    global _variant
    assert v in ("bf16", "f16")
    _variant = v


def variant():
    return _variant


def load(v=None):
    v = v or _variant
    lib = _libs.get(v)
    if lib is not None:
        return lib
    path = LIB_PATH if v == "bf16" else LIB_PATH_F16
    if not os.path.exists(path):
        raise RuntimeError(
            f"{path} is missing: build it with `make -C xmc-gan_amd/csrc` (or __graft_entry__.build()). "
            "The XMC-GAN step has no CPU/PyTorch fallback.")
    lib = C.CDLL(path)
    for name, args in _SIGS.items():
        fn = getattr(lib, name)
        fn.argtypes = args
        fn.restype = _RESTYPE.get(name, C.c_int)
    if lib.xmc_abi_version() != ABI_VERSION:
        raise RuntimeError(f"{path}: ABI version {lib.xmc_abi_version()}, this binding needs {ABI_VERSION} (stale build?)")
    if lib.xmc_half_format() != (0 if v == "bf16" else 1):
        raise RuntimeError(f"{path} was not built for the {v} storage format")
    lib.xmc_set_prezeroed(1)
    _libs[v] = lib
    return lib


_ECODES = {-1: "XMC_EINVAL (bad argument)", -2: "XMC_EALIGN (alignment / channel multiple)", -3: "XMC_ESHAPE (shape out of range)"}


def check(rc, what):
    if rc != 0:
        msg = _ECODES.get(rc) or (f"hipError_t {-rc - 1000}" if rc <= -1000 else f"unexpected return code {rc}")
        raise XmcHipError(f"{what} failed: {msg}")


def call(name, *args):
    lib = load()
    check(getattr(lib, name)(*args), name)
```

xmc-gan_amd/ops/_engine.py:

```python
import ctypes as C
import weakref
import torch
from .. import lib as L
from .. import prof
from ._config import (
    _DEBUG_DISPATCH, _code, _nbytes, _need_cuda, _p, _st, _weights_epoch, bump_weights_epoch, chan_pad, pad_to)


class ConvGeom:

    __slots__ = ("cin", "cout", "k", "s", "p", "row_perm", "_perm_dev", "groups", "kh", "kw", "ph", "pw")

    def __init__(self, cin, cout, k=1, s=1, p=0, row_perm=None, groups=1):
        self.kh, self.kw = k if isinstance(k, (tuple, list)) else (k, k)
        self.ph, self.pw = p if isinstance(p, (tuple, list)) else (p, p)
        assert self.kh >= 1 and self.kw >= 1 and self.kh * self.kw <= 127 and s >= 1
        assert cin % groups == 0 and cout % groups == 0
        self.cin, self.cout, self.s = cin, cout, s
        self.k = self.kh if self.kh == self.kw else None
        self.p = self.ph if self.ph == self.pw else None
        self.groups = groups
        self.row_perm = row_perm
        self._perm_dev = None

    @property
    def ntaps(self):
        return self.kh * self.kw

    def out_hw(self, h, w):
        return (h + 2 * self.ph - self.kh) // self.s + 1, (w + 2 * self.pw - self.kw) // self.s + 1

    def taps(self):
        return [(i - self.ph, j - self.pw, i * self.kw + j) for i in range(self.kh) for j in range(self.kw)]

    def perm_dev(self, device):
        if self.row_perm is None:
            return None
        if self._perm_dev is None or self._perm_dev.device != device:
            self._perm_dev = torch.as_tensor(self.row_perm, dtype=torch.int32, device=device).contiguous()
        return self._perm_dev


def _igemm(d, what):
    lib = L.load()
    nb = lib.xmc_conv_splitk_ws_bytes(C.byref(d))
    if nb > 0:
        ws = torch.empty(nb, dtype=torch.uint8, device=torch.cuda.current_device())
        d.splitk_ws, d.splitk_ws_bytes = ws.data_ptr(), nb
    L.check(lib.xmc_conv_igemm(C.byref(d), _st()), what)


def _fill_taps(d, cls, taps):
    for t, (dh, dw, wi) in enumerate(taps):
        d.dh[cls][t] = dh
        d.dw[cls][t] = dw
        d.wi[cls][t] = wi


_pack_cache = {}


class _PackEntry:
    __slots__ = ("ref", "version", "pepoch", "gepoch", "geom", "out", "up", "transpose", "wf", "private", "born", "lo")

    def valid(self, w, geom):
        return (self.ref() is w and self.version == w._version and self.pepoch == getattr(w, "_xmc_epoch", 0) and
                self.gepoch == _weights_epoch[0] and self.geom is geom)


def _pack_shape(geom, transpose, dtype, up):
    cs_p = chan_pad(geom.cin, dtype)
    cd_p = pad_to(geom.cout, 8)
    rows, cols = (pad_to(cs_p, 32), cd_p) if transpose else (pad_to(cd_p, 32), cs_p)
    return (16 if up else geom.ntaps), rows, cols


def _pack_job(wf, out, geom, transpose, up, lo=False):
    j = L.PackJob()
    j.lo = int(bool(lo))
    j.w, j.wpk = wf.data_ptr(), out.data_ptr()
    perm = None if up else geom.perm_dev(wf.device)
    j.row_perm = perm.data_ptr() if perm is not None else None
    j.Co, j.Ci, j.KHW = geom.cout, geom.cin, geom.ntaps
    j.rows_pad, j.cols_pad = out.shape[1], out.shape[2]
    j.transpose, j.dtype, j.groups, j.upconv = int(transpose), _code(out.dtype), (1 if up else geom.groups), int(up)
    return j


def _pack(w, geom, transpose, dtype, up=False, lo=False):
    assert not up or geom.groups == 1
    assert not lo or dtype != torch.float32
    out = torch.empty(_pack_shape(geom, transpose, dtype, up), dtype=dtype, device=w.device)
    wf = w.detach()
    if wf.dtype != torch.float32 or not wf.is_contiguous():
        wf = wf.float().contiguous()
    job = _pack_job(wf, out, geom, transpose, up, lo)
    L.check(L.load().xmc_pack_weight_multi(C.byref(job), 1, _st()), "xmc_pack_weight_multi")
    return out


def _packed_cached(w, geom, transpose, dtype, up=False, lo=False):
    if not isinstance(w, torch.nn.Parameter):
        return _pack(w, geom, transpose, dtype, up, lo)
    k = (id(w), "lo" if lo else bool(up), int(transpose), dtype)
    hit = _pack_cache.get(k)
    if hit is not None and hit.valid(w, geom):
        return hit.out
    e = _PackEntry()
    e.ref, e.geom, e.up, e.transpose, e.lo = weakref.ref(w), geom, bool(up), int(transpose), bool(lo)
    e.version, e.pepoch, e.gepoch = w._version, getattr(w, "_xmc_epoch", 0), _weights_epoch[0]
    wd = w.detach()
    e.wf = wd if (wd.dtype == torch.float32 and wd.is_contiguous()) else None
    e.out = _pack(w, geom, transpose, dtype, up, lo)
    e.private = w.is_cuda and torch.cuda.is_current_stream_capturing()
    _pack_serial[0] += 1
    e.born = _pack_serial[0]
    if hit is not None and _graphs_alive[0]:
        _retired_packs.append(hit.out)
    _pack_cache[k] = e
    return e.out


def _packed_upconv_cached(w, geom, transpose, dtype):
    return _packed_cached(w, geom, transpose, dtype, up=True)


_graphs_alive = [0]
_retired_packs = []
_pack_serial = [0]


def end_of_capture(failed=False):
    if failed:
        for k in [k for k, e in _pack_cache.items() if e.private]:
            del _pack_cache[k]
        bump_weights_epoch()
        return _pack_serial[0]
    _graphs_alive[0] += 1
    for k in [k for k, e in _pack_cache.items() if e.private]:
        del _pack_cache[k]
    return _pack_serial[0]


def drop_packs_newer_than(serial):
    if _pack_serial[0] == serial:
        return serial
    for k in [k for k, e in _pack_cache.items() if e.born > serial]:
        if _graphs_alive[0]:
            _retired_packs.append(_pack_cache[k].out)
        del _pack_cache[k]
    return _pack_serial[0]


def graph_released():
    _graphs_alive[0] = max(0, _graphs_alive[0] - 1)
    if _graphs_alive[0] == 0:
        _retired_packs.clear()


def repack_params(params):
    ids = {id(p): p for p in params}
    jobs, ents = [], []
    for k in [k for k, e in _pack_cache.items() if e.ref() is None]:
        if _graphs_alive[0]:
            _retired_packs.append(_pack_cache[k].out)
        del _pack_cache[k]
    for (pid, _up, _tr, _dt), e in _pack_cache.items():
        w = ids.get(pid)
        if w is None or e.ref() is not w or e.wf is None or e.gepoch != _weights_epoch[0] or e.version != w._version:
            continue
        if e.wf.data_ptr() != w.data_ptr():
            continue
        jobs.append(_pack_job(e.wf, e.out, e.geom, e.transpose, e.up, e.lo))
        ents.append((e, w))
    if not jobs:
        return 0
    arr = (L.PackJob * len(jobs))(*jobs)
    L.check(L.load().xmc_pack_weight_multi(arr, len(jobs), _st()), "xmc_pack_weight_multi")
    for e, w in ents:
        e.pepoch = getattr(w, "_xmc_epoch", 0)
    return len(jobs)


def _cast_raw(x, dtype):
    if x.dtype == dtype:
        return x
    x = x.contiguous()
    y = torch.empty_like(x, dtype=dtype)
    L.call("xmc_cast", _p(x), _p(y), x.numel(), _code(x.dtype), _code(dtype), _st())
    return y


def _upconv_fwd_raw(x, w, bias, geom, act, out_dtype):
    _need_cuda(x, w)
    assert geom.k == 3 and geom.s == 1 and geom.p == 1
    N, H, W, CS = x.shape
    cd_p = pad_to(geom.cout, 8)
    wpk = _packed_upconv_cached(w, geom, 0, x.dtype)
    y = torch.empty((N, 2 * H, 2 * W, cd_p), dtype=out_dtype, device=x.device)
    d = L.ConvDesc()
    d.src, d.wpk, d.dst = x.data_ptr(), wpk.data_ptr(), y.data_ptr()
    d.bias = bias.data_ptr() if bias is not None else None
    d.N, d.SH, d.SW, d.CS = N, H, W, CS
    d.DH, d.DW, d.CD = 2 * H, 2 * W, cd_p
    d.MH, d.MW, d.SA, d.DA, d.src_shift = H, W, 1, 2, 0
    d.ntaps, d.nclass, d.CDw = 4, 4, wpk.shape[1]
    d.act, d.dtype, d.out_dtype = act, _code(x.dtype), _code(out_dtype)
    for i in range(2):
        for j in range(2):
            cls = i * 2 + j
            _fill_taps(d, cls, [(i - 1 + th, j - 1 + tw, cls * 4 + th * 2 + tw) for th in range(2) for tw in range(2)])
            d.dph[cls], d.dpw[cls] = i, j
    with prof.launch("igemm_kernel (conv fwd+dgrad, MFMA implicit GEMM)", 2.0 * N * 4 * H * W * geom.cout * geom.cin * 9,
                     f"upconv-fwd {x.dtype} N{N} {2 * H}x{2 * W} {geom.cin}->{geom.cout} k3s1", _nbytes(x, wpk, y)):
        _igemm(d, "xmc_conv_igemm(upconv fwd)")
    return y


def _upconv_dgrad_raw(dy, w, geom, in_dtype):
    _need_cuda(dy, w)
    N, OH, OW, CDy = dy.shape
    H, W = OH // 2, OW // 2
    cs_p = chan_pad(geom.cin, in_dtype)
    wpk = _packed_upconv_cached(w, geom, 1, dy.dtype)
    dx = torch.empty((N, H, W, cs_p), dtype=in_dtype, device=dy.device)
    d = L.ConvDesc()
    d.src, d.wpk, d.dst = dy.data_ptr(), wpk.data_ptr(), dx.data_ptr()
    d.N, d.SH, d.SW, d.CS = N, OH, OW, CDy
    d.DH, d.DW, d.CD = H, W, cs_p
    d.MH, d.MW, d.SA, d.DA, d.src_shift = H, W, 2, 1, 0
    d.ntaps, d.nclass, d.CDw = 16, 1, wpk.shape[1]
    d.act, d.dtype, d.out_dtype = L.ACT_NONE, _code(dy.dtype), _code(in_dtype)
    taps = []
    for i in range(2):
        for th in range(2):
            ro = i - 2 * (i - 1 + th)
            for j in range(2):
                for tw in range(2):
                    co = j - 2 * (j - 1 + tw)
                    taps.append((ro, co, (i * 2 + j) * 4 + th * 2 + tw))
    _fill_taps(d, 0, taps)
    with prof.launch("igemm_kernel (conv fwd+dgrad, MFMA implicit GEMM)", 2.0 * N * OH * OW * geom.cout * geom.cin * 9,
                     f"upconv-dgrad {dy.dtype} N{N} {OH}x{OW} {geom.cin}->{geom.cout} k3s1", _nbytes(dy, wpk, dx)):
        _igemm(d, "xmc_conv_igemm(upconv dgrad)")
    return dx


def _conv_fwd_raw(x, w, bias, geom, act, out_dtype, res=None, alpha=None, up=False, res_mode=0, want2=False, want_pool=False,
                  round_act=False, mask=None, out=None, post_act=L.ACT_NONE, want_sign=False, sc_img=None, w_lo=False, taps=None):
    _need_cuda(x, w)
    table = geom.taps() if taps is None else geom.taps()[taps[0]:taps[1]]
    assert 1 <= len(table) <= L.MAX_TAPS, (geom.kh, geom.kw, taps)
    N, H, W, CS = x.shape
    sh = 1 if up else 0
    Hv, Wv = H << sh, W << sh
    OH, OW = geom.out_hw(Hv, Wv)
    cd_p = pad_to(geom.cout, 8)
    assert CS == chan_pad(geom.cin, x.dtype), (CS, geom.cin)
    wpk = _packed_cached(w, geom, 0, x.dtype, lo=w_lo)
    if out is None:
        y = torch.empty((N, OH, OW, cd_p), dtype=out_dtype, device=x.device)
    else:
        assert tuple(out.shape) == (N, OH, OW, cd_p) and out.dtype == out_dtype and out.is_contiguous() and out.device == x.device
        y = out
    d = L.ConvDesc()
    d.src, d.wpk, d.dst = x.data_ptr(), wpk.data_ptr(), y.data_ptr()
    d.bias = bias.data_ptr() if bias is not None else None
    d.res = res.data_ptr() if res is not None else None
    d.alpha_dev = alpha.data_ptr() if alpha is not None else None
    d.N, d.SH, d.SW, d.CS = N, H, W, CS
    d.DH, d.DW, d.CD = OH, OW, cd_p
    d.MH, d.MW, d.SA, d.DA, d.src_shift = OH, OW, geom.s, 1, sh
    d.ntaps, d.nclass, d.CDw = len(table), 1, wpk.shape[1]
    d.act, d.dtype, d.out_dtype = act, _code(x.dtype), _code(out_dtype)
    d.res_mode, d.round_act = res_mode, int(bool(round_act))
    d.groups = geom.groups
    d.post_act = post_act
    _fill_taps(d, 0, table)
    if bias is not None:
        assert bias.dtype == torch.float32 and bias.numel() >= cd_p, "bias must be f32 and padded to the stored channels"
    if res is not None:
        want = (N, OH // 2, OW // 2, cd_p) if res_mode == 2 else tuple(y.shape)
        assert tuple(res.shape) == want and res.dtype == out_dtype and res.is_contiguous(), (res.shape, want)
    if mask is not None:
        assert mask.shape == y.shape and mask.dtype == out_dtype and mask.is_contiguous()
        d.mask = mask.data_ptr()
    outs = [y]
    if want2:
        y2 = torch.empty_like(y)
        d.dst2 = y2.data_ptr()
        outs.append(y2)
    if want_sign:
        assert not want2
        bits = torch.empty((N, OH, OW, cd_p // 8), dtype=torch.uint8, device=x.device)
        d.sign_bits = bits.data_ptr()
        outs.append(bits)
    if want_pool:
        assert OH % 2 == 0 and OW % 2 == 0 and out_dtype == x.dtype
        yp = torch.empty((N, OH // 2, OW // 2, cd_p), dtype=out_dtype, device=x.device)
        d.dst_pool = yp.data_ptr()
        outs.append(yp)
    if sc_img is not None:
        img, frag, sbias = sc_img
        assert res is None and tuple(img.shape) == (N, 2 * OH, 2 * OW, 8) and img.dtype == x.dtype and img.is_contiguous()
        d.sc_img, d.sc_frag, d.sc_bias = img.data_ptr(), frag.data_ptr(), sbias.data_ptr()
        with prof.launch("igemm_kernel (conv fwd+dgrad, MFMA implicit GEMM)", 2.0 * N * OH * OW * geom.cout * (geom.cin * geom.k * geom.k + 48),
                         f"fwd+sc {x.dtype} N{N} {H}x{W} {geom.cin}->{geom.cout} k{geom.k}s{geom.s}", _nbytes(x, wpk, img, *outs)):
            rc = L.load().xmc_conv_ptile_scimg(C.byref(d), _st())
        if rc == 1:
            return None
        L.check(rc, "xmc_conv_ptile_scimg")
        return y if len(outs) == 1 else tuple(outs)
    with prof.launch("igemm_kernel (conv fwd+dgrad, MFMA implicit GEMM)", 2.0 * N * OH * OW * geom.cout * geom.cin * len(table),
                     f"fwd {x.dtype} N{N} {H}x{W} {geom.cin}->{geom.cout} k{geom.k or f'{geom.kh}x{geom.kw}'}s{geom.s}", _nbytes(x, wpk, res, mask, *outs)):
        _igemm(d, "xmc_conv_igemm(fwd)")
    return y if len(outs) == 1 else tuple(outs)


def _conv1x1_pair_raw(x, w, bias, geom, out_dtype):
    _need_cuda(x, w)
    assert geom.k == 1 and geom.s == 1 and geom.p == 0 and geom.groups == 1
    N, H, W, CS = x.shape
    cd_p = pad_to(geom.cout, 8)
    if "no_pw1x1_split" not in _DEBUG_DISPATCH:
        wpk, wlo = _packed_cached(w, geom, 0, x.dtype), _packed_cached(w, geom, 0, x.dtype, lo=True)
        y = torch.empty((N, H, W, cd_p), dtype=out_dtype, device=x.device)
        d = L.ConvDesc()
        d.src, d.wpk, d.wpk_lo, d.dst = x.data_ptr(), wpk.data_ptr(), wlo.data_ptr(), y.data_ptr()
        d.bias = bias.data_ptr() if bias is not None else None
        d.N, d.SH, d.SW, d.CS = N, H, W, CS
        d.DH, d.DW, d.CD = H, W, cd_p
        d.MH, d.MW, d.SA, d.DA, d.src_shift = H, W, 1, 1, 0
        d.ntaps, d.nclass, d.CDw = 1, 1, wpk.shape[1]
        d.act, d.dtype, d.out_dtype = L.ACT_NONE, _code(x.dtype), _code(out_dtype)
        _fill_taps(d, 0, [(0, 0, 0)])
        with prof.launch("igemm_kernel (conv fwd+dgrad, MFMA implicit GEMM)", 2.0 * N * H * W * geom.cout * geom.cin,
                         f"fwd-pair {x.dtype} N{N} {H}x{W} {geom.cin}->{geom.cout} k1s1", _nbytes(x, wpk, wlo, y)):
            rc = L.load().xmc_conv_pw1x1_split(C.byref(d), _st())
        if rc == 0:
            return y
        if rc != 1:
            L.check(rc, "xmc_conv_pw1x1_split")
    y32 = _conv_fwd_raw(_cast_raw(x, torch.float32), w, bias, geom, L.ACT_NONE, torch.float32)
    return _cast_raw(y32, out_dtype)


class _StagedMask:

    def __init__(self, dy, bits):
        assert bits.dtype == torch.uint8 and bits.numel() * 8 == dy.numel() and dy.is_contiguous()
        self.dy, self.bits, self._full = dy, bits, None

    def materialised(self):
        if self._full is None:
            self._full = torch.empty_like(self.dy)
            L.call("xmc_signmask_apply", _p(self.dy), _p(self.bits), _p(self._full), self.dy.numel(), 0.2, _code(self.dy.dtype), _st())
        return self._full


def _conv_dgrad_raw(dy, w, geom, in_hw, in_dtype, mask=None, res=None, res_rows=False, res_scale=1.0, alpha=None, want_sumpool=False,
                    dot=None, src_bits=None):
    staged = dy if isinstance(dy, _StagedMask) else None
    if staged is not None:
        dy = staged.dy
    d, dx, dxp, wpk = _dgrad_desc(dy, w, geom, in_hw, in_dtype, mask, res, res_rows, res_scale, alpha, want_sumpool, dot)
    N, OH, OW, CDy = dy.shape
    H, W = in_hw
    if src_bits is not None:
        assert geom.k == 1 and geom.s == 1 and not want_sumpool and src_bits.dtype == torch.uint8 and src_bits.numel() * 8 == dy.numel()
        dym = torch.empty_like(dy)
        with prof.launch("igemm_kernel (conv fwd+dgrad, MFMA implicit GEMM)", 2.0 * N * OH * OW * geom.cout * geom.cin,
                         f"dgrad+srcmask {dy.dtype} N{N} {H}x{W} {geom.cin}->{geom.cout} k1s1", _nbytes(dy, wpk, dx, dym)):
            rc = L.load().xmc_conv_pw1x1_masked_src(C.byref(d), _p(src_bits), _p(dym), 0.2, _st())
            if rc == 1:
                _igemm(d, "xmc_conv_igemm(dgrad)")
                L.call("xmc_signmask_apply", _p(dy), _p(src_bits), _p(dym), dy.numel(), 0.2, _code(dy.dtype), _st())
            else:
                L.check(rc, "xmc_conv_pw1x1_masked_src")
        return dx, dym
    if staged is not None:
        d.mask_bits = staged.bits.data_ptr()
        with prof.launch("igemm_kernel (conv fwd+dgrad, MFMA implicit GEMM)", 2.0 * N * OH * OW * geom.cout * geom.cin * geom.k * geom.k,
                         f"dgrad+bits {dy.dtype} N{N} {H}x{W} {geom.cin}->{geom.cout} k{geom.k}s{geom.s}", _nbytes(dy, wpk, dx, mask, res, dxp)):
            rc = L.load().xmc_conv_ptile_bits(C.byref(d), _st())
        if rc == 0:
            return (dx, dxp) if want_sumpool else dx
        if rc != 1:
            L.check(rc, "xmc_conv_ptile_bits")
        d.mask_bits, d.src = None, staged.materialised().data_ptr()
    with prof.launch("igemm_kernel (conv fwd+dgrad, MFMA implicit GEMM)", 2.0 * N * OH * OW * geom.cout * geom.cin * geom.k * geom.k,
                     f"dgrad {dy.dtype} N{N} {H}x{W} {geom.cin}->{geom.cout} k{geom.k}s{geom.s}", _nbytes(dy, wpk, dx, mask, res, dxp)):
        _igemm(d, "xmc_conv_igemm(dgrad)")
    return (dx, dxp) if want_sumpool else dx


def _dgrad_desc(dy, w, geom, in_hw, in_dtype, mask=None, res=None, res_rows=False, res_scale=1.0, alpha=None, want_sumpool=False, dot=None):
    _need_cuda(dy, w)
    N, OH, OW, CDy = dy.shape
    H, W = in_hw
    assert CDy == pad_to(geom.cout, 8)
    cs_p = chan_pad(geom.cin, in_dtype)
    wpk = _packed_cached(w, geom, 1, dy.dtype)
    if cs_p % 8:
        raise RuntimeError("dgrad destination needs a channel count that is a multiple of 8")
    dx = torch.empty((N, H, W, cs_p), dtype=in_dtype, device=dy.device)
    d = L.ConvDesc()
    d.src, d.wpk, d.dst = dy.data_ptr(), wpk.data_ptr(), dx.data_ptr()
    d.N, d.SH, d.SW, d.CS = N, OH, OW, CDy
    d.DH, d.DW, d.CD = H, W, cs_p
    s, k, p = geom.s, geom.k, geom.p
    assert k is not None and p is not None and k % s == 0 and k * k <= L.MAX_TAPS, "data gradient: square kernel, k % s == 0"
    d.MH, d.MW, d.SA, d.DA, d.src_shift = H // s, W // s, 1, s, 0
    d.nclass, d.CDw = s * s, wpk.shape[1]
    d.act, d.dtype, d.out_dtype = L.ACT_NONE, _code(dy.dtype), _code(in_dtype)
    d.groups = geom.groups
    assert H % s == 0 and W % s == 0
    ntaps = None
    for ph in range(s):
        for pw in range(s):
            cls = ph * s + pw
            taps = [((ph + p - kh) // s, (pw + p - kw) // s, kh * k + kw)
                    for kh in range(k) if (ph + p - kh) % s == 0
                    for kw in range(k) if (pw + p - kw) % s == 0]
            assert ntaps in (None, len(taps))
            ntaps = len(taps)
            _fill_taps(d, cls, taps)
            d.dph[cls], d.dpw[cls] = ph, pw
    d.ntaps = ntaps
    if alpha is not None:
        d.alpha_dev = alpha.data_ptr()
    if mask is not None:
        assert mask.shape == dx.shape and mask.dtype == dx.dtype and mask.is_contiguous()
        d.mask = mask.data_ptr()
    if dot is not None:
        assert mask is not None and dot.dtype == torch.float32 and dot.numel() == 1
        d.dot = dot.data_ptr()
    if res is not None:
        want = (N, H // s, W // s, cs_p) if res_rows else tuple(dx.shape)
        assert tuple(res.shape) == want and res.dtype == dx.dtype and res.is_contiguous(), (res.shape, want)
        assert not res_rows or s == 2
        d.res, d.res_mode, d.res_scale = res.data_ptr(), 1 if res_rows else 0, float(res_scale)
    dxp = None
    if want_sumpool:
        assert s == 1 and H % 2 == 0 and W % 2 == 0 and in_dtype == dy.dtype
        dxp = torch.empty((N, H // 2, W // 2, cs_p), dtype=in_dtype, device=dy.device)
        d.dst_pool, d.pool_scale = dxp.data_ptr(), 1.0
    return d, dx, dxp, wpk


class _ZeroArena:

    def __init__(self):
        self.buf, self.off, self.need, self.retired, self.active = {}, {}, {}, [], set()

    def new_iteration(self, device):
        key = (device.type, device.index)
        need = self.need.get(key, 0)
        buf = self.buf.get(key)
        capturing = device.type == "cuda" and torch.cuda.is_current_stream_capturing()
        if need and (buf is None or buf.numel() < need) and not capturing:
            if buf is not None:
                self.retired.append(buf)
            buf = self.buf[key] = torch.empty(int(need * 1.05) + 1024, dtype=torch.float32, device=device)
        elif buf is not None and need and need < buf.numel() // 2 and not capturing and not _graphs_alive[0]:
            buf = self.buf[key] = torch.empty(int(need * 1.05) + 1024, dtype=torch.float32, device=device)
        if buf is not None:
            buf.zero_()
        self.off[key], self.need[key] = 0, 0
        self.active.add(key)

    def end_iteration(self, device):
        self.active.discard((device.type, device.index))

    def zeros(self, shape, device):
# ... 356 lines not shown
```

xmc-gan_amd/optim.py:

```python
import collections
import ctypes as C

import torch

from . import lib as L
from . import ops


class HipAdam(torch.optim.Optimizer):
    def __init__(self, params, lr=1e-3, betas=(0.9, 0.999), eps=1e-8):
        super().__init__(params, dict(lr=lr, betas=betas, eps=eps, weight_decay=0, amsgrad=False))
        self._tables = collections.OrderedDict()
        self._chunk = None
        self._arenas, self._arena_off = [], 0
        self._free = {}

    MAX_TABLES = 8

    def _pinned(self, nbytes):
        free = self._free.get(nbytes)
        if free:
            return free.pop()
        if not self._arenas or self._arena_off + nbytes > self._arenas[-1].numel():
            if torch.cuda.is_current_stream_capturing():
                raise RuntimeError("HipAdam: pinned staging arena exhausted during graph capture; run a warm-up step first")
            total = sum(p.numel() for g in self.param_groups for p in g["params"])
            nparams = sum(len(g["params"]) for g in self.param_groups)
            per_table = 64 * nparams + 8 * (total // 4096 + nparams) + 256
            self._arenas.append(torch.empty(max(16 * per_table, nbytes), dtype=torch.uint8).pin_memory())
            self._arena_off = 0
        out = self._arenas[-1][self._arena_off: self._arena_off + nbytes]
        self._arena_off += nbytes
        return out

    def _state_for(self, p):
        st = self.state[p]
        if not st:
            st["step"] = torch.zeros(1, dtype=torch.int32, device=p.device)
            st["exp_avg"] = torch.zeros_like(p, dtype=torch.float32, memory_format=torch.contiguous_format)
            st["exp_avg_sq"] = torch.zeros_like(p, dtype=torch.float32, memory_format=torch.contiguous_format)
        return st

    def state_dict(self):
        sd = super().state_dict()
        sd["state"] = {k: {**st, "step": st["step"].detach().to("cpu", torch.float32).reshape(())} if "step" in st else st
                       for k, st in sd["state"].items()}
        return sd

    def load_state_dict(self, state_dict):
        for g in state_dict["param_groups"]:
            if g.get("weight_decay", 0) != 0 or g.get("amsgrad", False) or g.get("maximize", False):
                raise ValueError("HipAdam implements Adam without weight decay / amsgrad / maximize (train_gan.py:483-484)")
        super().load_state_dict(state_dict)
        for p, st in self.state.items():
            if "step" in st:
                st["step"] = torch.as_tensor(st["step"]).detach().reshape(1).round().to(device=p.device, dtype=torch.int32)
            for k in ("exp_avg", "exp_avg_sq"):
                if k in st:
                    st[k] = st[k].to(device=p.device, dtype=torch.float32).contiguous()
        self._tables.clear()

    def _table(self, ps, device):
        key = tuple((p.data_ptr(), p.grad.data_ptr()) for p in ps)
        hit = self._tables.get(key)
        if hit is not None:
            self._tables.move_to_end(key)
            return hit[:4]
        if self._chunk is None:
            self._chunk = L.load().xmc_adam_chunk_elems()
        ents = (L.AdamEntry * len(ps))()
        chunks = []
        for i, p in enumerate(ps):
            st = self._state_for(p)
            g = p.grad
            if g.dtype != torch.float32 or not g.is_contiguous() or not p.is_contiguous():
                raise RuntimeError("HipAdam needs contiguous f32 parameters and gradients")
            ents[i].param, ents[i].grad = p.data_ptr(), g.data_ptr()
            ents[i].m, ents[i].v = st["exp_avg"].data_ptr(), st["exp_avg_sq"].data_ptr()
            ents[i].step, ents[i].n = st["step"].data_ptr(), p.numel()
            chunks += [(i, c) for c in range((p.numel() + self._chunk - 1) // self._chunk)]
        raw = bytes(ents)
        chb = torch.tensor(chunks, dtype=torch.int32).numpy().tobytes()
        n0, n1 = (len(raw) + 63) // 64 * 64, (len(chb) + 63) // 64 * 64
        tab_h, ch_h = self._pinned(n0), self._pinned(n1)
        tab_h[: len(raw)].copy_(torch.frombuffer(bytearray(raw), dtype=torch.uint8))
        ch_h[: len(chb)].copy_(torch.frombuffer(bytearray(chb), dtype=torch.uint8))
        tab = tab_h.to(device, non_blocking=True)
        ch = ch_h.to(device, non_blocking=True).view(torch.int32)
        capturing = torch.cuda.is_current_stream_capturing()
        self._tables[key] = (tab, ch, len(ps), len(chunks), tab_h, ch_h, capturing)
        if len(self._tables) > self.MAX_TABLES and not capturing:
            torch.cuda.current_stream().synchronize()
            for k in list(self._tables):
                if len(self._tables) <= self.MAX_TABLES:
                    break
                ent = self._tables[k]
                if k != key and not ent[6]:
                    del self._tables[k]
                    for h in (ent[4], ent[5]):
                        self._free.setdefault(h.numel(), []).append(h)
        return self._tables[key][:4]

    @torch.no_grad()
    def step(self, closure=None, grad_scale=1.0, scaler=None, ema=None):
        assert closure is None
        if ema is not None:
            return self._step_ema(grad_scale, scaler, ema)
        groups = []
        for group in self.param_groups:
            ps = [p for p in group["params"] if p.grad is not None]
            if not ps:
                continue
            if not ps[0].is_cuda:
                raise RuntimeError("HipAdam runs on the GPU only (no CPU fallback)")
            groups.append((group, self._table(ps, ps[0].device)))
        st = C.c_void_p(torch.cuda.current_stream().cuda_stream) if groups else None
        if scaler is None:
            for group, (tab, ch, nt, nc) in groups:
                b1, b2 = group["betas"]
                L.call("xmc_adam_step", C.c_void_p(tab.data_ptr()), nt, C.c_void_p(ch.data_ptr()), nc,
                       float(group["lr"]), float(b1), float(b2), float(group["eps"]), float(grad_scale), st)
        else:
            assert grad_scale == 1.0
            CHECK, UPDATE, RESCALE = 1, 2, 4
            passes = [CHECK | UPDATE] if len(groups) == 1 else [CHECK, UPDATE]
            for mode in passes:
                for gi, (group, (tab, ch, nt, nc)) in enumerate(groups):
                    b1, b2 = group["betas"]
                    m = mode | (RESCALE if (mode & UPDATE) and gi == len(groups) - 1 else 0)
                    L.call("xmc_adam_step_scaled", C.c_void_p(tab.data_ptr()), nt, C.c_void_p(ch.data_ptr()), nc,
                           float(group["lr"]), float(b1), float(b2), float(group["eps"]), C.c_void_p(scaler.sf.data_ptr()),
                           C.c_void_p(scaler.si.data_ptr()), m, scaler.growth, scaler.backoff, scaler.interval, st)
        self._repack()

    def _repack(self):
        changed = [p for group in self.param_groups for p in group["params"] if p.grad is not None]
        for p in changed:
            p._xmc_epoch = getattr(p, "_xmc_epoch", 0) + 1
        ops.repack_params(changed)

    def _step_ema(self, grad_scale, scaler, ema):
        groups, fused = [], set()
        for group in self.param_groups:
            ps = [p for p in group["params"] if p.grad is not None]
            if not ps:
                continue
            if not ps[0].is_cuda:
                raise RuntimeError("HipAdam runs on the GPU only (no CPU fallback)")
            groups.append((group, self._table(ps, ps[0].device), ema._table(ps, fused=True)))
            fused.update(id(p) for p in ps)
        rest = [p for p in ema.params if id(p) not in fused]
        st = C.c_void_p(torch.cuda.current_stream().cuda_stream)
        nupd = C.c_void_p(ema.num_updates.data_ptr())
        decay, start = float(ema.decay), int(ema.start)
        flag = C.c_void_p(scaler.si.data_ptr()) if scaler is not None else None
        CHECK, UPDATE, RESCALE = 1, 2, 4
        one_call = len(groups) == 1 and not rest
        if scaler is not None:
            assert grad_scale == 1.0
        if scaler is not None and not one_call:
            for group, (tab, ch, nt, nc), _ in groups:
                b1, b2 = group["betas"]
                L.call("xmc_adam_step_scaled", C.c_void_p(tab.data_ptr()), nt, C.c_void_p(ch.data_ptr()), nc,
                       float(group["lr"]), float(b1), float(b2), float(group["eps"]), C.c_void_p(scaler.sf.data_ptr()),
                       flag, CHECK, scaler.growth, scaler.backoff, scaler.interval, st)
        if rest:
            etab, ech, ent, enc = ema._table(rest)
            L.call("xmc_ema_step", C.c_void_p(etab.data_ptr()), ent, C.c_void_p(ech.data_ptr()), enc, decay, start, nupd, flag,
                   0 if groups else 1, st)
        for gi, (group, (tab, ch, nt, nc), (etab, _, _, _)) in enumerate(groups):
            b1, b2 = group["betas"]
            last = gi == len(groups) - 1
            if scaler is None:
                L.call("xmc_adam_ema_step", C.c_void_p(tab.data_ptr()), C.c_void_p(etab.data_ptr()), nt, C.c_void_p(ch.data_ptr()), nc,
                       float(group["lr"]), float(b1), float(b2), float(group["eps"]), float(grad_scale), decay, start, nupd,
                       1 if last else 0, st)
            else:
                L.call("xmc_adam_ema_step_scaled", C.c_void_p(tab.data_ptr()), C.c_void_p(etab.data_ptr()), nt,
                       C.c_void_p(ch.data_ptr()), nc, float(group["lr"]), float(b1), float(b2), float(group["eps"]),
                       C.c_void_p(scaler.sf.data_ptr()), flag, (CHECK if one_call else 0) | UPDATE | (RESCALE if last else 0), scaler.growth, scaler.backoff,
                       scaler.interval, decay, start, nupd, 1 if last else 0, st)
        self._repack()


class ParamEMA:

    def __init__(self, module, decay, start=0):
        decay, start = float(decay), int(start)
        if not 0.0 <= decay < 1.0:
            raise ValueError(f"ParamEMA: decay must be in [0, 1), got {decay}")
        if start < 0:
            raise ValueError(f"ParamEMA: start must be >= 0, got {start}")
        self.decay, self.start = decay, start
        self.source = module
        self.names, self.params = [], []
        for name, p in module.named_parameters():
            if p.dtype != torch.float32 or not p.is_contiguous():
                raise RuntimeError(f"ParamEMA needs contiguous f32 parameters ({name})")
            self.names.append(name)
            self.params.append(p)
        if not self.params:
            raise ValueError("ParamEMA: the module has no parameters")
        self.shadow = [p.detach().clone(memory_format=torch.contiguous_format) for p in self.params]
        self._shadow_of = {id(p): e for p, e in zip(self.params, self.shadow)}
        device = self.params[0].device
        self.num_updates = torch.zeros(1, dtype=torch.int32, device=device)
        self._tables = {}
        self._chunk = None
        self._arenas, self._arena_off = [], 0
        if device.type == "cuda":
            self._pinned(0)

    def _pinned(self, nbytes):
        if not self._arenas or self._arena_off + nbytes > self._arenas[-1].numel():
            if torch.cuda.is_current_stream_capturing():
                raise RuntimeError("ParamEMA: pinned staging arena exhausted during graph capture; run a warm-up step first")
            total = sum(p.numel() for p in self.params)
            per_table = 32 * len(self.params) + 8 * (total // 4096 + len(self.params)) + 256
            self._arenas.append(torch.empty(max(8 * per_table, nbytes), dtype=torch.uint8).pin_memory())
            self._arena_off = 0
        out = self._arenas[-1][self._arena_off: self._arena_off + nbytes]
        self._arena_off += nbytes
        return out

    def _table(self, ps, fused=False):
        with_params = not fused
        key = (tuple(p.data_ptr() for p in ps), with_params)
        hit = self._tables.get(key)
        if hit is not None:
            return hit[:4]
        device = ps[0].device
        if device.type != "cuda":
            raise RuntimeError("ParamEMA runs on the GPU only (no CPU fallback)")
        if self._chunk is None:
            self._chunk = L.load().xmc_adam_chunk_elems()
        ents = (L.EmaEntry * len(ps))()
        chunks = []
        for i, p in enumerate(ps):
            e = self._shadow_of.get(id(p))
            if e is None and with_params:
                raise RuntimeError("ParamEMA: not a parameter of the averaged module")
            ents[i].shadow, ents[i].param, ents[i].n = (e.data_ptr() if e is not None else None), p.data_ptr(), p.numel()
            chunks += [(i, c) for c in range((p.numel() + self._chunk - 1) // self._chunk)]
        raw = bytes(ents)
        chb = torch.tensor(chunks, dtype=torch.int32).numpy().tobytes() if with_params else b""
        n0, n1 = (len(raw) + 63) // 64 * 64, (len(chb) + 63) // 64 * 64
        tab_h, ch_h = self._pinned(n0), self._pinned(n1)
        tab_h[: len(raw)].copy_(torch.frombuffer(bytearray(raw), dtype=torch.uint8))
        tab = tab_h.to(device, non_blocking=True)
        ch = None
        if with_params:
            ch_h[: len(chb)].copy_(torch.frombuffer(bytearray(chb), dtype=torch.uint8))
            ch = ch_h.to(device, non_blocking=True).view(torch.int32)
        self._tables[key] = (tab, ch, len(ps), len(chunks), tab_h, ch_h)
        return self._tables[key][:4]

    @torch.no_grad()
    def update(self, skip_flag=None):
        tab, ch, nt, nc = self._table(self.params)
        L.call("xmc_ema_step", C.c_void_p(tab.data_ptr()), nt, C.c_void_p(ch.data_ptr()), nc, float(self.decay), int(self.start),
               C.c_void_p(self.num_updates.data_ptr()), C.c_void_p(skip_flag.data_ptr()) if skip_flag is not None else None, 1,
               C.c_void_p(torch.cuda.current_stream().cuda_stream))

    def state_dict(self):
        return {"shadow": {n: e.detach().clone() for n, e in zip(self.names, self.shadow)},
                "num_updates": int(self.num_updates.item()), "decay": self.decay, "start": self.start}

    @torch.no_grad()
    def load_state_dict(self, sd):
        missing = [n for n in self.names if n not in sd["shadow"]]
        if missing:
            raise KeyError(f"ParamEMA.load_state_dict: no shadow for {missing}")
        for n, e in zip(self.names, self.shadow):
            e.copy_(sd["shadow"][n])
        self.num_updates.fill_(int(sd["num_updates"]))
        if "decay" in sd:
            self.decay = float(sd["decay"])
        if "start" in sd:
            self.start = int(sd["start"])

    @torch.no_grad()
    def copy_to(self, module):
        targets = dict(module.named_parameters())
        if set(targets) != set(self.names):
            raise KeyError("ParamEMA.copy_to: the module's parameters are not those of the averaged module")
        for n, e in zip(self.names, self.shadow):
            targets[n].copy_(e)
        src = dict(self.source.named_buffers())
        for n, b in module.named_buffers():
            b.copy_(src[n])
        return module
```

Measured before the change: 6378 images/s.

## Fuse conv weight repacking into the Adam update kernel via LDS tiles

Adds a tiled Adam path in which each workgroup updates a tile of a conv weight tensor, stages the updated values in LDS, and writes the packed or transposed bf16/f32 copies used by the conv kernels directly. Those packed copies are then skipped by the separate repack pass. This removes a second full read of the parameters and the repack kernel launches after each optimizer step. In exchange the kernel is more complex, the tiled path gathers rows strided through a row permutation, it needs more LDS, and the table build now depends on the pack metadata.

```diff
diff --git a/include/xmc_gan_hip.h b/include/xmc_gan_hip.h
--- a/include/xmc_gan_hip.h
+++ b/include/xmc_gan_hip.h
@@ -250,6 +250,26 @@
 int xmc_adam_step_scaled(const XmcAdamEntry* table_dev, int ntensors, const int32_t* chunks_dev, int nchunks,
                          float lr, float beta1, float beta2, float eps, float* scale_dev, int32_t* flags_dev,
                          int mode, float growth, float backoff, int interval, void* stream);
+#define XMC_ADAM_PACK_MAX 6
+typedef struct XmcAdamPackTensor {
+    int32_t tensor;
+    int32_t Co, Ci, KHW;
+    int32_t ncopies, reserved;
+    const int32_t* row_perm;
+    XmcPackJob copy[XMC_ADAM_PACK_MAX];
+} XmcAdamPackTensor;
+typedef struct XmcAdamTile {
+    int32_t ptensor;
+    int32_t r0, ci0, vec16;
+} XmcAdamTile;
+int xmc_adam_tile_dims(int KHW, int32_t* CB, int32_t* CIB);
+int xmc_adam_pack_step(const XmcAdamEntry* table_dev, int ntensors, const int32_t* chunks_dev, int nchunks,
+                       const XmcAdamPackTensor* ptens_dev, const XmcAdamTile* tiles_dev, int ntiles,
+                       float lr, float beta1, float beta2, float eps, float grad_scale, void* stream);
+int xmc_adam_pack_step_scaled(const XmcAdamEntry* table_dev, int ntensors, const int32_t* chunks_dev, int nchunks, int nchunks_all,
+                              const XmcAdamPackTensor* ptens_dev, const XmcAdamTile* tiles_dev, int ntiles,
+                              float lr, float beta1, float beta2, float eps, float* scale_dev, int32_t* flags_dev,
+                              int mode, float growth, float backoff, int interval, void* stream);
 
 typedef struct XmcEmaEntry {
     float* shadow;
diff --git a/xmc-gan_amd/csrc/adam.hip b/xmc-gan_amd/csrc/adam.hip
--- a/xmc-gan_amd/csrc/adam.hip
+++ b/xmc-gan_amd/csrc/adam.hip
@@ -39,38 +39,203 @@
     si[0] = 0;
 }
 
-__global__ void adam_kernel(const XmcAdamEntry* __restrict__ tab, const int2* __restrict__ chunks,
-                            float lr, float b1, float b2, float eps, float gs, const float* __restrict__ sf,
-                            const int* __restrict__ si) {
+template <bool FMA>
+__device__ __forceinline__ float adam_elem(float P, float G, float& M, float& V, float b1, float b2, float step_size, float bc2s,
+                                           float eps) {
+#pragma clang fp contract(off)
+    const float t = (1.f - b1) * G, u = ((1.f - b2) * G) * G;
+    M = FMA ? __builtin_fmaf(b1, M, t) : b1 * M + t;
+    V = FMA ? __builtin_fmaf(b2, V, u) : b2 * V + u;
+    return P - (step_size * M) / (sqrtf(V) / bc2s + eps);
+}
+struct AdamCoef { float b1, b2, eps, step_size, bc2s, gs; };
+
+template <int KHW> struct TileDims;
+template <> struct TileDims<1> { static constexpr int CB = 64, CIB = 64; };
+template <> struct TileDims<9> { static constexpr int CB = 32, CIB = 32; };
+template <> struct TileDims<16> { static constexpr int CB = 16, CIB = 32; };
+template <int KHW> constexpr int tile_lds_floats() { return KHW * TileDims<KHW>::CB * (TileDims<KHW>::CIB + 1); }
+constexpr int TILE_LDS_BYTES = 4 * (tile_lds_floats<9>() > tile_lds_floats<16>() ? tile_lds_floats<9>() : tile_lds_floats<16>());
+static_assert(tile_lds_floats<1>() * 4 <= TILE_LDS_BYTES && TILE_LDS_BYTES <= 40 * 1024, "four workgroups per CU");
+
+template <int KHW, bool FMA>
+__device__ __forceinline__ void tile_update(float* __restrict__ lds, const XmcAdamEntry& e, const XmcAdamPackTensor& pt,
+                                            const XmcAdamTile& tl, const AdamCoef& k) {
+    constexpr int CB = TileDims<KHW>::CB, CIB = TileDims<KHW>::CIB, PC = CIB + 1, RUN = CIB * KHW;
+    static_assert(RUN % 4 == 0, "a full run is a whole number of 16-byte accesses");
+    const int rows = pt.Co - tl.r0 < CB ? pt.Co - tl.r0 : CB, cib = pt.Ci - tl.ci0 < CIB ? pt.Ci - tl.ci0 : CIB;
+    const int run = cib * KHW;
+    const int64_t pitch = (int64_t)pt.Ci * KHW, col0 = (int64_t)tl.ci0 * KHW;
+    float* __restrict__ p = e.param; const float* __restrict__ g = e.grad; float* __restrict__ m = e.m; float* __restrict__ v = e.v;
+    if (tl.vec16) {
+        constexpr int RUN4 = RUN / 4;
+        const int run4 = run >> 2;
+        for (int u = threadIdx.x; u < CB * RUN4; u += NT) {
+            const int r = u / RUN4, j = u - r * RUN4;
+            if (r >= rows) break;
+            if (j >= run4) continue;
+            const int srow = pt.row_perm ? pt.row_perm[tl.r0 + r] : tl.r0 + r;
+            const int64_t off = srow * pitch + col0 + 4 * j;
+            f32x4 P = *reinterpret_cast<f32x4*>(p + off), G = *reinterpret_cast<const f32x4*>(g + off);
+            f32x4 M = *reinterpret_cast<f32x4*>(m + off), V = *reinterpret_cast<f32x4*>(v + off);
+#pragma unroll
+            for (int q = 0; q < 4; ++q) {
+                float Mq = M[q], Vq = V[q];
+                P[q] = adam_elem<FMA>(P[q], G[q] * k.gs, Mq, Vq, k.b1, k.b2, k.step_size, k.bc2s, k.eps);
+                M[q] = Mq; V[q] = Vq;
+            }
+            *reinterpret_cast<f32x4*>(p + off) = P; *reinterpret_cast<f32x4*>(m + off) = M; *reinterpret_cast<f32x4*>(v + off) = V;
+#pragma unroll
+            for (int q = 0; q < 4; ++q) {
+                const int el = 4 * j + q, ci = el / KHW, t = el - ci * KHW;
+                lds[(t * CB + r) * PC + ci] = P[q];
+            }
+        }
+    } else {
+        for (int u = threadIdx.x; u < CB * RUN; u += NT) {
+            const int r = u / RUN, el = u - r * RUN;
+            if (r >= rows) break;
+            if (el >= run) continue;
+            const int srow = pt.row_perm ? pt.row_perm[tl.r0 + r] : tl.r0 + r;
+            const int64_t off = srow * pitch + col0 + el;
+            float M = m[off], V = v[off];
+            const float P = adam_elem<FMA>(p[off], g[off] * k.gs, M, V, k.b1, k.b2, k.step_size, k.bc2s, k.eps);
+            p[off] = P; m[off] = M; v[off] = V;
+            const int ci = el / KHW, t = el - ci * KHW;
+            lds[(t * CB + r) * PC + ci] = P;
+        }
+    }
+}
+
+__device__ __forceinline__ void tile_store8(const XmcPackJob& job, int64_t idx, const float (&val)[8], int nv, bool lo) {
+    if (job.dtype == XMC_BF16) {
+        xmc_h16* d = reinterpret_cast<xmc_h16*>(job.wpk) + idx;
+        if (nv == 8 && (reinterpret_cast<uintptr_t>(d) & 15) == 0) {
+            bf16x8 h;
+#pragma unroll
+            for (int i = 0; i < 8; ++i) h[i] = xmc_pack_round16(val[i], lo);
+            *reinterpret_cast<bf16x8*>(d) = h;
+        } else {
+#pragma unroll
+            for (int i = 0; i < 8; ++i)
+                if (i < nv) d[i] = xmc_pack_round16(val[i], lo);
+        }
+    } else {
+        float* d = reinterpret_cast<float*>(job.wpk) + idx;
+        if (nv == 8 && (reinterpret_cast<uintptr_t>(d) & 15) == 0) {
+            f32x4 a, b;
+#pragma unroll
+            for (int i = 0; i < 4; ++i) { a[i] = val[i]; b[i] = val[4 + i]; }
+            reinterpret_cast<f32x4*>(d)[0] = a; reinterpret_cast<f32x4*>(d)[1] = b;
+        } else {
+#pragma unroll
+            for (int i = 0; i < 8; ++i)
+                if (i < nv) d[i] = val[i];
+        }
+    }
+}
+
+template <int KHW, bool TR>
+__device__ __forceinline__ void tile_pack_copy(const float* __restrict__ lds, const XmcPackJob& job, const XmcAdamTile& tl, int rows, int cib) {
+    constexpr int CB = TileDims<KHW>::CB, CIB = TileDims<KHW>::CIB, PC = CIB + 1;
+    constexpr int OCT = (TR ? CB : CIB) / 8, OTH = TR ? CIB : CB, LI = TR ? PC : 1;
+    static_assert((OCT & (OCT - 1)) == 0 && (OTH & (OTH - 1)) == 0, "unit decodes are shifts");
+    const int64_t plane = (int64_t)job.rows_pad * job.cols_pad;
+    const bool up = KHW == 9 && job.upconv != 0;
+    const int na = TR ? rows : cib, nb = TR ? cib : rows;
+    const int units = (up ? 4 : KHW) * OTH * OCT;
+    for (int u = threadIdx.x; u < units; u += NT) {
+        const int a = u % OCT, b = (u / OCT) % OTH, t = u / (OCT * OTH);
+        const int nv = na - 8 * a < 8 ? na - 8 * a : 8;
+        if (b >= nb || nv <= 0) continue;
+        const int l0 = TR ? 8 * a * PC + b : b * PC + 8 * a;
+        const int64_t pos = TR ? (int64_t)(tl.ci0 + b) * job.cols_pad + tl.r0 + 8 * a : (int64_t)(tl.r0 + b) * job.cols_pad + tl.ci0 + 8 * a;
+        float val[8];
+        if constexpr (KHW == 9) {
+            if (up) {
+                float w9[8][9];
+#pragma unroll
+                for (int i = 0; i < 8; ++i)
+#pragma unroll
+                    for (int q = 0; q < 9; ++q) w9[i][q] = lds[q * CB * PC + l0 + i * LI];
+#pragma unroll
+                for (int s = 0; s < 4; ++s) {
+#pragma unroll
+                    for (int i = 0; i < 8; ++i) val[i] = xmc_upconv_slice(w9[i], 4 * t + s);
+                    tile_store8(job, (4 * t + s) * plane + pos, val, nv, false);
+                }
+                continue;
+            }
+        }
+#pragma unroll
+        for (int i = 0; i < 8; ++i) val[i] = lds[t * CB * PC + l0 + i * LI];
+        tile_store8(job, t * plane + pos, val, nv, job.lo != 0);
+    }
+}
+
+template <int KHW>
+__device__ __forceinline__ void tile_pack(const float* __restrict__ lds, const XmcAdamPackTensor& pt, const XmcAdamTile& tl) {
+    constexpr int CB = TileDims<KHW>::CB, CIB = TileDims<KHW>::CIB;
+    const int rows = pt.Co - tl.r0 < CB ? pt.Co - tl.r0 : CB, cib = pt.Ci - tl.ci0 < CIB ? pt.Ci - tl.ci0 : CIB;
+    for (int c = 0; c < pt.ncopies; ++c) {
+        if (pt.copy[c].transpose) tile_pack_copy<KHW, true>(lds, pt.copy[c], tl, rows, cib);
+        else tile_pack_copy<KHW, false>(lds, pt.copy[c], tl, rows, cib);
+    }
+}
+
+template <int KHW>
+__device__ __forceinline__ void tile_chunk(float* lds, const XmcAdamEntry& e, const XmcAdamPackTensor& pt, const XmcAdamTile& tl,
+                                           const AdamCoef& k) {
+    if ((e.n & 3) == 0) tile_update<KHW, true>(lds, e, pt, tl, k);
+    else tile_update<KHW, false>(lds, e, pt, tl, k);
+    __syncthreads();
+    tile_pack<KHW>(lds, pt, tl);
+}
+
+__global__ __launch_bounds__(NT) void adam_kernel(const XmcAdamEntry* __restrict__ tab, const int2* __restrict__ chunks, int nchunks,
+                                                  const XmcAdamPackTensor* __restrict__ ptens, const XmcAdamTile* __restrict__ tiles,
+                                                  float lr, float b1, float b2, float eps, float gs, const float* __restrict__ sf,
+                                                  const int* __restrict__ si) {
+    extern __shared__ float tile_lds[];
     if (si && *si) return;
     if (sf) gs *= sf[1];
-    const int2 c = chunks[blockIdx.x];
-    const XmcAdamEntry e = tab[c.x];
+    const bool flat = (int)blockIdx.x < nchunks;
+    int2 c = make_int2(0, 0);
+    XmcAdamTile tl = {0, 0, 0, 0};
+    if (flat) c = chunks[blockIdx.x];
+    else tl = tiles[(int)blockIdx.x - nchunks];
+    const XmcAdamEntry e = tab[flat ? c.x : ptens[tl.ptensor].tensor];
     const int t = *e.step + 1;
     const float bc1 = 1.f - powf(b1, (float)t), bc2s = sqrtf(1.f - powf(b2, (float)t));
     const float step_size = lr / bc1;
+    if (!flat) {
+        const AdamCoef k = {b1, b2, eps, step_size, bc2s, gs};
+        const XmcAdamPackTensor& pt = ptens[tl.ptensor];
+        if (pt.KHW == 9) tile_chunk<9>(tile_lds, e, pt, tl, k);
+        else if (pt.KHW == 16) tile_chunk<16>(tile_lds, e, pt, tl, k);
+        else tile_chunk<1>(tile_lds, e, pt, tl, k);
+        return;
+    }
     const int64_t base = (int64_t)c.y * CHUNK;
     const int64_t lim = e.n - base < CHUNK ? e.n - base : CHUNK;
     float* p = e.param + base; const float* g = e.grad + base; float* m = e.m + base; float* v = e.v + base;
     if ((e.n & 3) == 0) {
         for (int i = threadIdx.x * 4; i < lim; i += NT * 4) {
-            f32x4 P = *reinterpret_cast<f32x4*>(p + i), G = *reinterpret_cast<const f32x4*>(g + i) * gs;
+            f32x4 P = *reinterpret_cast<f32x4*>(p + i), G = *reinterpret_cast<const f32x4*>(g + i);
             f32x4 M = *reinterpret_cast<f32x4*>(m + i), V = *reinterpret_cast<f32x4*>(v + i);
 #pragma unroll
-            for (int k = 0; k < 4; ++k) {
-                M[k] = b1 * M[k] + (1.f - b1) * G[k];
-                V[k] = b2 * V[k] + (1.f - b2) * G[k] * G[k];
-                P[k] -= step_size * M[k] / (sqrtf(V[k]) / bc2s + eps);
+            for (int q = 0; q < 4; ++q) {
+                float Mq = M[q], Vq = V[q];
+                P[q] = adam_elem<true>(P[q], G[q] * gs, Mq, Vq, b1, b2, step_size, bc2s, eps);
+                M[q] = Mq; V[q] = Vq;
             }
             *reinterpret_cast<f32x4*>(p + i) = P; *reinterpret_cast<f32x4*>(m + i) = M; *reinterpret_cast<f32x4*>(v + i) = V;
         }
     } else {
         for (int i = threadIdx.x; i < lim; i += NT) {
-            float G = g[i] * gs;
-            float M = b1 * m[i] + (1.f - b1) * G;
-            float V = b2 * v[i] + (1.f - b2) * G * G;
-            p[i] -= step_size * M / (sqrtf(V) / bc2s + eps);
-            m[i] = M; v[i] = V;
+            float M = m[i], V = v[i];
+            const float P = adam_elem<false>(p[i], g[i] * gs, M, V, b1, b2, step_size, bc2s, eps);
+            p[i] = P; m[i] = M; v[i] = V;
         }
     }
 }
@@ -83,13 +248,61 @@
 
 extern "C" int xmc_adam_chunk_elems(void) { return CHUNK; }
 
+extern "C" int xmc_adam_tile_dims(int KHW, int32_t* CB, int32_t* CIB) {
+    if (!CB || !CIB) return XMC_EINVAL;
+    if (KHW == 1) { *CB = TileDims<1>::CB; *CIB = TileDims<1>::CIB; }
+    else if (KHW == 9) { *CB = TileDims<9>::CB; *CIB = TileDims<9>::CIB; }
+    else if (KHW == 16) { *CB = TileDims<16>::CB; *CIB = TileDims<16>::CIB; }
+    else return XMC_EINVAL;
+    return 0;
+}
+
+namespace {
+bool pack_args_ok(const void* table_dev, int ntensors, const void* chunks_dev, int nchunks, int nchunks_all, const void* ptens_dev,
+                  const void* tiles_dev, int ntiles) {
+    if (!table_dev || ntensors < 1 || nchunks < 0 || nchunks_all < nchunks || ntiles < 0 || nchunks + ntiles < 1) return false;
+    if (nchunks_all > 0 && !chunks_dev) return false;
+    return ntiles == 0 || (ptens_dev && tiles_dev);
+}
+void launch_adam(hipStream_t st, const XmcAdamEntry* table_dev, const int32_t* chunks_dev, int nchunks, const XmcAdamPackTensor* ptens_dev,
+                 const XmcAdamTile* tiles_dev, int ntiles, float lr, float b1, float b2, float eps, float gs, const float* sf, const int* si) {
+    hipLaunchKernelGGL(adam_kernel, dim3(nchunks + ntiles), dim3(NT), ntiles ? TILE_LDS_BYTES : 0, st, table_dev,
+                       reinterpret_cast<const int2*>(chunks_dev), nchunks, ptens_dev, tiles_dev, lr, b1, b2, eps, gs, sf, si);
+}
+}
+
+extern "C" int xmc_adam_pack_step(const XmcAdamEntry* table_dev, int ntensors, const int32_t* chunks_dev, int nchunks,
+                                  const XmcAdamPackTensor* ptens_dev, const XmcAdamTile* tiles_dev, int ntiles,
+                                  float lr, float beta1, float beta2, float eps, float grad_scale, void* stream) {
+    if (!pack_args_ok(table_dev, ntensors, chunks_dev, nchunks, nchunks, ptens_dev, tiles_dev, ntiles)) return XMC_EINVAL;
+    hipStream_t st = reinterpret_cast<hipStream_t>(stream);
+    launch_adam(st, table_dev, chunks_dev, nchunks, ptens_dev, tiles_dev, ntiles, lr, beta1, beta2, eps, grad_scale, nullptr, nullptr);
+    hipLaunchKernelGGL(adam_bump_kernel, dim3((ntensors + NT - 1) / NT), dim3(NT), 0, st, table_dev, ntensors, (const int*)nullptr);
+    XMC_LAUNCH_CHECK();
+    return 0;
+}
+
 extern "C" int xmc_adam_step(const XmcAdamEntry* table_dev, int ntensors, const int32_t* chunks_dev, int nchunks,
                              float lr, float beta1, float beta2, float eps, float grad_scale, void* stream) {
-    if (!table_dev || !chunks_dev || ntensors < 1 || nchunks < 1) return XMC_EINVAL;
+    if (!chunks_dev || nchunks < 1) return XMC_EINVAL;
+    return xmc_adam_pack_step(table_dev, ntensors, chunks_dev, nchunks, nullptr, nullptr, 0, lr, beta1, beta2, eps, grad_scale, stream);
+}
+
+extern "C" int xmc_adam_pack_step_scaled(const XmcAdamEntry* table_dev, int ntensors, const int32_t* chunks_dev, int nchunks, int nchunks_all,
+                                         const XmcAdamPackTensor* ptens_dev, const XmcAdamTile* tiles_dev, int ntiles,
+                                         float lr, float beta1, float beta2, float eps, float* scale_dev, int32_t* flags_dev,
+                                         int mode, float growth, float backoff, int interval, void* stream) {
+    if (!pack_args_ok(table_dev, ntensors, chunks_dev, nchunks, nchunks_all, ptens_dev, tiles_dev, ntiles) || nchunks_all < 1 || !scale_dev ||
+        !flags_dev || interval < 1 || (mode & 7) == 0)
+        return XMC_EINVAL;
     hipStream_t st = reinterpret_cast<hipStream_t>(stream);
-    hipLaunchKernelGGL(adam_kernel, dim3(nchunks), dim3(NT), 0, st, table_dev, reinterpret_cast<const int2*>(chunks_dev), lr, beta1, beta2, eps,
-                       grad_scale, (const float*)nullptr, (const int*)nullptr);
-    hipLaunchKernelGGL(adam_bump_kernel, dim3((ntensors + NT - 1) / NT), dim3(NT), 0, st, table_dev, ntensors, (const int*)nullptr);
+    if (mode & XMC_ADAM_CHECK)
+        hipLaunchKernelGGL(adam_check_kernel, dim3(nchunks_all), dim3(NT), 0, st, table_dev, reinterpret_cast<const int2*>(chunks_dev), flags_dev);
+    if (mode & XMC_ADAM_UPDATE) {
+        launch_adam(st, table_dev, chunks_dev, nchunks, ptens_dev, tiles_dev, ntiles, lr, beta1, beta2, eps, 1.f, scale_dev, flags_dev);
+        hipLaunchKernelGGL(adam_bump_kernel, dim3((ntensors + NT - 1) / NT), dim3(NT), 0, st, table_dev, ntensors, (const int*)flags_dev);
+    }
+    if (mode & XMC_ADAM_RESCALE) hipLaunchKernelGGL(scaler_update_kernel, dim3(1), dim3(64), 0, st, scale_dev, flags_dev, growth, backoff, interval);
     XMC_LAUNCH_CHECK();
     return 0;
 }
@@ -97,18 +310,9 @@
 extern "C" int xmc_adam_step_scaled(const XmcAdamEntry* table_dev, int ntensors, const int32_t* chunks_dev, int nchunks,
                                     float lr, float beta1, float beta2, float eps, float* scale_dev, int32_t* flags_dev,
                                     int mode, float growth, float backoff, int interval, void* stream) {
-    if (!table_dev || !chunks_dev || ntensors < 1 || nchunks < 1 || !scale_dev || !flags_dev || interval < 1 || (mode & 7) == 0) return XMC_EINVAL;
-    hipStream_t st = reinterpret_cast<hipStream_t>(stream);
-    const int2* ch = reinterpret_cast<const int2*>(chunks_dev);
-    if (mode & XMC_ADAM_CHECK) hipLaunchKernelGGL(adam_check_kernel, dim3(nchunks), dim3(NT), 0, st, table_dev, ch, flags_dev);
-    if (mode & XMC_ADAM_UPDATE) {
-        hipLaunchKernelGGL(adam_kernel, dim3(nchunks), dim3(NT), 0, st, table_dev, ch, lr, beta1, beta2, eps, 1.f, (const float*)scale_dev,
-                           (const int*)flags_dev);
-        hipLaunchKernelGGL(adam_bump_kernel, dim3((ntensors + NT - 1) / NT), dim3(NT), 0, st, table_dev, ntensors, (const int*)flags_dev);
-    }
-    if (mode & XMC_ADAM_RESCALE) hipLaunchKernelGGL(scaler_update_kernel, dim3(1), dim3(64), 0, st, scale_dev, flags_dev, growth, backoff, interval);
-    XMC_LAUNCH_CHECK();
-    return 0;
+    if (!chunks_dev || nchunks < 1) return XMC_EINVAL;
+    return xmc_adam_pack_step_scaled(table_dev, ntensors, chunks_dev, nchunks, nchunks, nullptr, nullptr, 0, lr, beta1, beta2, eps, scale_dev,
+                                     flags_dev, mode, growth, backoff, interval, stream);
 }
 
 namespace {
@@ -137,16 +341,6 @@
         }
     }
     for (int i = body + threadIdx.x; i < lim; i += NT) e[i] = ema_elem(e[i], p[i], w, copy);
-}
-
-template <bool FMA>
-__device__ __forceinline__ float adam_elem(float P, float G, float& M, float& V, float b1, float b2, float step_size, float bc2s,
-                                           float eps) {
-#pragma clang fp contract(off)
-    const float t = (1.f - b1) * G, u = ((1.f - b2) * G) * G;
-    M = FMA ? __builtin_fmaf(b1, M, t) : b1 * M + t;
-    V = FMA ? __builtin_fmaf(b2, V, u) : b2 * V + u;
-    return P - (step_size * M) / (sqrtf(V) / bc2s + eps);
 }
 
 template <bool FMA>
diff --git a/xmc-gan_amd/csrc/common.h b/xmc-gan_amd/csrc/common.h
--- a/xmc-gan_amd/csrc/common.h
+++ b/xmc-gan_amd/csrc/common.h
@@ -106,6 +106,20 @@
     return __builtin_bit_cast(u32x4, h);
 }
 
+__device__ __forceinline__ xmc_h16 xmc_pack_round16(float v, bool lo) { return lo ? (xmc_h16)(v - (float)(xmc_h16)v) : (xmc_h16)v; }
+__device__ __forceinline__ float xmc_upconv_slice(const float (&w9)[9], int sl) {
+    const int i = sl >> 3, j = (sl >> 2) & 1, th = (sl >> 1) & 1, tw = sl & 1;
+    const int kh0 = (i == 0) ? (th == 0 ? 0 : 1) : (th == 0 ? 0 : 2), kh1 = (i == 0) ? (th == 0 ? 0 : 2) : (th == 0 ? 1 : 2);
+    const int kw0 = (j == 0) ? (tw == 0 ? 0 : 1) : (tw == 0 ? 0 : 2), kw1 = (j == 0) ? (tw == 0 ? 0 : 2) : (tw == 0 ? 1 : 2);
+    float v = 0.f;
+#pragma unroll
+    for (int kh = 0; kh < 3; ++kh)
+#pragma unroll
+        for (int kw = 0; kw < 3; ++kw)
+            if (kh >= kh0 && kh <= kh1 && kw >= kw0 && kw <= kw1) v += w9[kh * 3 + kw];
+    return v;
+}
+
 template <int DT> struct Vec8;
 template <> struct Vec8<XMC_BF16> {
     static constexpr int BYTES = 16;
diff --git a/xmc-gan_amd/csrc/pointwise.hip b/xmc-gan_amd/csrc/pointwise.hip
--- a/xmc-gan_amd/csrc/pointwise.hip
+++ b/xmc-gan_amd/csrc/pointwise.hip
@@ -524,7 +524,7 @@
 struct PackJobs { XmcPackJob j[XMC_PACK_MULTI_MAX]; int32_t first[XMC_PACK_MULTI_MAX + 1]; int32_t njobs; };
 template <int DT>
 __device__ __forceinline__ void pack_store(void* p, int64_t i, float v, bool lo = false) {
-    if (DT == XMC_BF16) reinterpret_cast<xmc_h16*>(p)[i] = lo ? (xmc_h16)(v - (float)(xmc_h16)v) : (xmc_h16)v;
+    if (DT == XMC_BF16) reinterpret_cast<xmc_h16*>(p)[i] = xmc_pack_round16(v, lo);
     else reinterpret_cast<float*>(p)[i] = v;
 }
 template <int DT>
@@ -538,18 +538,7 @@
 #pragma unroll
         for (int t = 0; t < 9; ++t) w9[t] = in ? job.w[((int64_t)co * job.Ci + ci) * 9 + t] : 0.f;
 #pragma unroll
-        for (int sl = 0; sl < 16; ++sl) {
-            const int i = sl >> 3, j = (sl >> 2) & 1, th = (sl >> 1) & 1, tw = sl & 1;
-            const int kh0 = (i == 0) ? (th == 0 ? 0 : 1) : (th == 0 ? 0 : 2), kh1 = (i == 0) ? (th == 0 ? 0 : 2) : (th == 0 ? 1 : 2);
-            const int kw0 = (j == 0) ? (tw == 0 ? 0 : 1) : (tw == 0 ? 0 : 2), kw1 = (j == 0) ? (tw == 0 ? 0 : 2) : (tw == 0 ? 1 : 2);
-            float v = 0.f;
-#pragma unroll
-            for (int kh = 0; kh < 3; ++kh)
-#pragma unroll
-                for (int kw = 0; kw < 3; ++kw)
-                    if (kh >= kh0 && kh <= kh1 && kw >= kw0 && kw <= kw1) v += w9[kh * 3 + kw];
-            pack_store<DT>(job.wpk, sl * plane + pos, v);
-        }
+        for (int sl = 0; sl < 16; ++sl) pack_store<DT>(job.wpk, sl * plane + pos, xmc_upconv_slice(w9, sl));
         return;
     }
     const int cog = job.Co / job.groups, cig = job.Ci / job.groups;
diff --git a/xmc-gan_amd/lib.py b/xmc-gan_amd/lib.py
--- a/xmc-gan_amd/lib.py
+++ b/xmc-gan_amd/lib.py
@@ -43,6 +43,18 @@
 
 class AdamEntry(C.Structure):
     _fields_ = [("param", vp), ("grad", vp), ("m", vp), ("v", vp), ("step", vp), ("n", i64)]
+
+
+ADAM_PACK_MAX = 6
+
+
+class AdamPackTensor(C.Structure):
+    _fields_ = [("tensor", i32), ("Co", i32), ("Ci", i32), ("KHW", i32), ("ncopies", i32), ("reserved", i32), ("row_perm", vp),
+                ("copy", PackJob * ADAM_PACK_MAX)]
+
+
+class AdamTile(C.Structure):
+    _fields_ = [("ptensor", i32), ("r0", i32), ("ci0", i32), ("vec16", i32)]
 
 
 class EmaEntry(C.Structure):
@@ -153,6 +165,9 @@
     "xmc_adam_chunk_elems": [],
     "xmc_adam_step": [vp, i32, vp, i32, f32, f32, f32, f32, f32, vp],
     "xmc_adam_step_scaled": [vp, i32, vp, i32, f32, f32, f32, f32, vp, vp, i32, f32, f32, i32, vp],
+    "xmc_adam_tile_dims": [i32, C.POINTER(i32), C.POINTER(i32)],
+    "xmc_adam_pack_step": [vp, i32, vp, i32, vp, vp, i32, f32, f32, f32, f32, f32, vp],
+    "xmc_adam_pack_step_scaled": [vp, i32, vp, i32, i32, vp, vp, i32, f32, f32, f32, f32, vp, vp, i32, f32, f32, i32, vp],
     "xmc_ema_step": [vp, i32, vp, i32, f32, i32, vp, vp, i32, vp],
     "xmc_adam_ema_step": [vp, vp, i32, vp, i32, f32, f32, f32, f32, f32, f32, i32, vp, i32, vp],
     "xmc_adam_ema_step_scaled": [vp, vp, i32, vp, i32, f32, f32, f32, f32, vp, vp, i32, f32, f32, i32, f32, i32, vp, i32, vp],
diff --git a/xmc-gan_amd/ops/_engine.py b/xmc-gan_amd/ops/_engine.py
--- a/xmc-gan_amd/ops/_engine.py
+++ b/xmc-gan_amd/ops/_engine.py
@@ -9,7 +9,7 @@
 
 class ConvGeom:
 
-    __slots__ = ("cin", "cout", "k", "s", "p", "row_perm", "_perm_dev", "groups", "kh", "kw", "ph", "pw")
+    __slots__ = ("cin", "cout", "k", "s", "p", "row_perm", "_perm_dev", "_perm_ok", "groups", "kh", "kw", "ph", "pw")
 
     def __init__(self, cin, cout, k=1, s=1, p=0, row_perm=None, groups=1):
         self.kh, self.kw = k if isinstance(k, (tuple, list)) else (k, k)
@@ -22,6 +22,7 @@
         self.groups = groups
         self.row_perm = row_perm
         self._perm_dev = None
+        self._perm_ok = None
 
     @property
     def ntaps(self):
@@ -32,6 +33,12 @@
 
     def taps(self):
         return [(i - self.ph, j - self.pw, i * self.kw + j) for i in range(self.kh) for j in range(self.kw)]
+
+    def perm_is_bijection(self):
+        if self._perm_ok is None:
+            perm = torch.as_tensor(self.row_perm).reshape(-1).to("cpu", torch.int64)
+            self._perm_ok = perm.numel() == self.cout and torch.equal(perm.sort().values, torch.arange(self.cout))
+        return self._perm_ok
 
     def perm_dev(self, device):
         if self.row_perm is None:
@@ -158,18 +165,49 @@
         _retired_packs.clear()
 
 
-def repack_params(params):
+def _bulk_entries(params):
     ids = {id(p): p for p in params}
+    for (pid, _up, _tr, _dt), e in _pack_cache.items():
+        w = ids.get(pid)
+        if w is None or e.ref() is not w or e.wf is None or e.gepoch != _weights_epoch[0] or e.version != w._version:
+            continue
+        if e.wf.data_ptr() != w.data_ptr():
+            continue
+        yield e, w
+
+
+def adam_pack_copies(params):
+    by_param = {}
+    for e, w in _bulk_entries(params):
+        by_param.setdefault(id(w), (w, []))[1].append(e)
+    out = {}
+    for pid, (w, es) in by_param.items():
+        g0 = es[0].geom
+        perms = {None if (e.up or e.geom.row_perm is None) else id(e.geom) for e in es}
+        if (len(es) > L.ADAM_PACK_MAX or len(perms) != 1 or w.dim() not in (2, 4) or g0.ntaps not in (1, 9, 16) or
+                any(e.geom.groups != 1 or e.geom.ntaps != g0.ntaps or (e.up and g0.ntaps != 9) for e in es) or
+                tuple(w.shape[:2]) != (g0.cout, g0.cin) or w.numel() != g0.cout * g0.cin * g0.ntaps or
+                any((e.geom.cout, e.geom.cin) != (g0.cout, g0.cin) for e in es)):
+            continue
+        if None not in perms and not next(e.geom for e in es if not e.up).perm_is_bijection():
+            continue
+        out[pid] = es
+    return out
+
+
+def adam_pack_job(e):
+    return _pack_job(e.wf, e.out, e.geom, e.transpose, e.up, e.lo)
+
+
+def repack_params(params, skip=()):
+    skip = {id(e) for e in skip}
     jobs, ents = [], []
     for k in [k for k, e in _pack_cache.items() if e.ref() is None]:
         if _graphs_alive[0]:
             _retired_packs.append(_pack_cache[k].out)
         del _pack_cache[k]
-    for (pid, _up, _tr, _dt), e in _pack_cache.items():
-        w = ids.get(pid)
-        if w is None or e.ref() is not w or e.wf is None or e.gepoch != _weights_epoch[0] or e.version != w._version:
-            continue
-        if e.wf.data_ptr() != w.data_ptr():
+    for e, w in _bulk_entries(params):
+        if id(e) in skip:
             continue
         jobs.append(_pack_job(e.wf, e.out, e.geom, e.transpose, e.up, e.lo))
         ents.append((e, w))
diff --git a/xmc-gan_amd/optim.py b/xmc-gan_amd/optim.py
--- a/xmc-gan_amd/optim.py
+++ b/xmc-gan_amd/optim.py
@@ -5,13 +5,34 @@
 
 from . import lib as L
 from . import ops
+
+
+def adam_chunk_tables(numels, packed, chunk, tile_dims):
+    flat, rest, order, tiles = [], [], [], []
+    for i, n in enumerate(numels):
+        pairs = [(i, c) for c in range((n + chunk - 1) // chunk)]
+        if i not in packed:
+            flat += pairs
+            continue
+        Co, Ci, KHW, addrs = packed[i]
+        CB, CIB = tile_dims[KHW]
+        assert n == Co * Ci * KHW and CIB % 4 == 0
+        rest += pairs
+        vec16 = int(all(a % 16 == 0 for a in addrs) and (Ci * KHW) % 4 == 0)
+        tiles += [(len(order), r0, ci0, vec16) for r0 in range(0, Co, CB) for ci0 in range(0, Ci, CIB)]
+        order.append(i)
+    return flat, rest, order, tiles
+
+
+class _Table:
+    __slots__ = ("tab", "ch", "nt", "nc", "nc_all", "pt", "tiles", "ntiles", "covered", "pinned", "capturing")
 
 
 class HipAdam(torch.optim.Optimizer):
     def __init__(self, params, lr=1e-3, betas=(0.9, 0.999), eps=1e-8):
         super().__init__(params, dict(lr=lr, betas=betas, eps=eps, weight_decay=0, amsgrad=False))
         self._tables = collections.OrderedDict()
-        self._chunk = None
+        self._chunk = self._dims = None
         self._arenas, self._arena_off = [], 0
         self._free = {}
 
@@ -27,6 +48,7 @@
             total = sum(p.numel() for g in self.param_groups for p in g["params"])
             nparams = sum(len(g["params"]) for g in self.param_groups)
             per_table = 64 * nparams + 8 * (total // 4096 + nparams) + 256
+            per_table += C.sizeof(L.AdamPackTensor) * nparams + C.sizeof(L.AdamTile) * (total // 1024 + 4 * nparams) + 128
             self._arenas.append(torch.empty(max(16 * per_table, nbytes), dtype=torch.uint8).pin_memory())
             self._arena_off = 0
         out = self._arenas[-1][self._arena_off: self._arena_off + nbytes]
@@ -60,16 +82,32 @@
                     st[k] = st[k].to(device=p.device, dtype=torch.float32).contiguous()
         self._tables.clear()
 
-    def _table(self, ps, device):
-        key = tuple((p.data_ptr(), p.grad.data_ptr()) for p in ps)
+    def _upload(self, raw, device):
+        n = (len(raw) + 63) // 64 * 64
+        h = self._pinned(n)
+        h[: len(raw)].copy_(torch.frombuffer(bytearray(raw), dtype=torch.uint8))
+        return h.to(device, non_blocking=True), h
+
+    def _tile_dims(self):
+        if self._dims is None:
+            self._dims = {}
+            for khw in (1, 9, 16):
+                cb, cib = C.c_int32(), C.c_int32()
+                L.call("xmc_adam_tile_dims", khw, C.byref(cb), C.byref(cib))
+                self._dims[khw] = (cb.value, cib.value)
+        return self._dims
+
+    def _table(self, ps, device, pack=False):
+        copies = ops.adam_pack_copies(ps) if pack else {}
+        key = tuple((p.data_ptr(), p.grad.data_ptr()) + tuple(e.out.data_ptr() for e in copies.get(id(p), ())) for p in ps)
         hit = self._tables.get(key)
-        if hit is not None:
+        if hit is not None and all(a is b for a, b in zip(hit.covered, (e for p in ps for e in copies.get(id(p), ())))):
             self._tables.move_to_end(key)
-            return hit[:4]
+            return hit
         if self._chunk is None:
             self._chunk = L.load().xmc_adam_chunk_elems()
         ents = (L.AdamEntry * len(ps))()
-        chunks = []
+        packed = {}
         for i, p in enumerate(ps):
             st = self._state_for(p)
             g = p.grad
@@ -78,34 +116,54 @@
             ents[i].param, ents[i].grad = p.data_ptr(), g.data_ptr()
             ents[i].m, ents[i].v = st["exp_avg"].data_ptr(), st["exp_avg_sq"].data_ptr()
             ents[i].step, ents[i].n = st["step"].data_ptr(), p.numel()
-            chunks += [(i, c) for c in range((p.numel() + self._chunk - 1) // self._chunk)]
-        raw = bytes(ents)
-        chb = torch.tensor(chunks, dtype=torch.int32).numpy().tobytes()
-        n0, n1 = (len(raw) + 63) // 64 * 64, (len(chb) + 63) // 64 * 64
-        tab_h, ch_h = self._pinned(n0), self._pinned(n1)
-        tab_h[: len(raw)].copy_(torch.frombuffer(bytearray(raw), dtype=torch.uint8))
-        ch_h[: len(chb)].copy_(torch.frombuffer(bytearray(chb), dtype=torch.uint8))
-        tab = tab_h.to(device, non_blocking=True)
-        ch = ch_h.to(device, non_blocking=True).view(torch.int32)
-        capturing = torch.cuda.is_current_stream_capturing()
-        self._tables[key] = (tab, ch, len(ps), len(chunks), tab_h, ch_h, capturing)
+            if id(p) in copies:
+                geom = copies[id(p)][0].geom
+                packed[i] = (geom.cout, geom.cin, geom.ntaps, (ents[i].param, ents[i].grad, ents[i].m, ents[i].v))
+        flat, rest, order, tiles = adam_chunk_tables([p.numel() for p in ps], packed, self._chunk, self._tile_dims() if packed else {})
+        t = _Table()
+        t.covered = [e for p in ps for e in copies.get(id(p), ())]
+        pts = (L.AdamPackTensor * max(len(order), 1))()
+        for k, i in enumerate(order):
+            es = copies[id(ps[i])]
+            pts[k].tensor, pts[k].ncopies = i, len(es)
+            pts[k].Co, pts[k].Ci, pts[k].KHW = packed[i][:3]
+            for c, e in enumerate(es):
+                pts[k].copy[c] = ops.adam_pack_job(e)
+            perm = [j.row_perm for j in pts[k].copy[: len(es)] if j.row_perm]
+            pts[k].row_perm = perm[0] if perm else None
+        tl = (L.AdamTile * max(len(tiles), 1))()
+        for k, (pt, r0, ci0, vec16) in enumerate(tiles):
+            tl[k].ptensor, tl[k].r0, tl[k].ci0, tl[k].vec16 = pt, r0, ci0, vec16
+        t.tab, h0 = self._upload(bytes(ents), device)
+        ch, h1 = self._upload(torch.tensor(flat + rest, dtype=torch.int32).numpy().tobytes(), device)
+        t.ch = ch.view(torch.int32)
+        t.pinned = [h0, h1]
+        t.pt = t.tiles = None
+        if tiles:
+            t.pt, h2 = self._upload(bytes(pts), device)
+            t.tiles, h3 = self._upload(bytes(tl), device)
+            t.pinned += [h2, h3]
+        t.nt, t.nc, t.nc_all, t.ntiles = len(ps), len(flat), len(flat) + len(rest), len(tiles)
+        t.capturing = capturing = torch.cuda.is_current_stream_capturing()
+        self._tables[key] = t
         if len(self._tables) > self.MAX_TABLES and not capturing:
             torch.cuda.current_stream().synchronize()
             for k in list(self._tables):
                 if len(self._tables) <= self.MAX_TABLES:
                     break
                 ent = self._tables[k]
-                if k != key and not ent[6]:
+                if k != key and not ent.capturing:
                     del self._tables[k]
-                    for h in (ent[4], ent[5]):
+                    for h in ent.pinned:
                         self._free.setdefault(h.numel(), []).append(h)
-        return self._tables[key][:4]
+        return t
 
     @torch.no_grad()
     def step(self, closure=None, grad_scale=1.0, scaler=None, ema=None):
         assert closure is None
         if ema is not None:
             return self._step_ema(grad_scale, scaler, ema)
+        pack = not ops.debug_switch("no_adam_pack")
         groups = []
         for group in self.param_groups:
             ps = [p for p in group["params"] if p.grad is not None]
@@ -113,31 +171,34 @@
                 continue
             if not ps[0].is_cuda:
                 raise RuntimeError("HipAdam runs on the GPU only (no CPU fallback)")
-            groups.append((group, self._table(ps, ps[0].device)))
+            groups.append((group, self._table(ps, ps[0].device, pack=pack)))
         st = C.c_void_p(torch.cuda.current_stream().cuda_stream) if groups else None
+        vp = lambda t: C.c_void_p(t.data_ptr()) if t is not None else None
         if scaler is None:
-            for group, (tab, ch, nt, nc) in groups:
+            for group, t in groups:
                 b1, b2 = group["betas"]
-                L.call("xmc_adam_step", C.c_void_p(tab.data_ptr()), nt, C.c_void_p(ch.data_ptr()), nc,
+                L.call("xmc_adam_pack_step", vp(t.tab), t.nt, vp(t.ch), t.nc, vp(t.pt), vp(t.tiles), t.ntiles,
                        float(group["lr"]), float(b1), float(b2), float(group["eps"]), float(grad_scale), st)
         else:
             assert grad_scale == 1.0
             CHECK, UPDATE, RESCALE = 1, 2, 4
             passes = [CHECK | UPDATE] if len(groups) == 1 else [CHECK, UPDATE]
             for mode in passes:
-                for gi, (group, (tab, ch, nt, nc)) in enumerate(groups):
+                for gi, (group, t) in enumerate(groups):
                     b1, b2 = group["betas"]
                     m = mode | (RESCALE if (mode & UPDATE) and gi == len(groups) - 1 else 0)
-                    L.call("xmc_adam_step_scaled", C.c_void_p(tab.data_ptr()), nt, C.c_void_p(ch.data_ptr()), nc,
+                    L.call("xmc_adam_pack_step_scaled", vp(t.tab), t.nt, vp(t.ch), t.nc, t.nc_all, vp(t.pt), vp(t.tiles), t.ntiles,
                            float(group["lr"]), float(b1), float(b2), float(group["eps"]), C.c_void_p(scaler.sf.data_ptr()),
                            C.c_void_p(scaler.si.data_ptr()), m, scaler.growth, scaler.backoff, scaler.interval, st)
-        self._repack()
-
-    def _repack(self):
+        self._repack([e for _, t in groups for e in t.covered])
+
+    def _repack(self, written=()):
         changed = [p for group in self.param_groups for p in group["params"] if p.grad is not None]
         for p in changed:
             p._xmc_epoch = getattr(p, "_xmc_epoch", 0) + 1
-        ops.repack_params(changed)
+        for e in written:
+            e.pepoch = e.ref()._xmc_epoch
+        ops.repack_params(changed, skip=written)
 
     def _step_ema(self, grad_scale, scaler, ema):
         groups, fused = [], set()
@@ -147,7 +208,8 @@
                 continue
             if not ps[0].is_cuda:
                 raise RuntimeError("HipAdam runs on the GPU only (no CPU fallback)")
-            groups.append((group, self._table(ps, ps[0].device), ema._table(ps, fused=True)))
+            t = self._table(ps, ps[0].device)
+            groups.append((group, (t.tab, t.ch, t.nt, t.nc), ema._table(ps, fused=True)))
             fused.update(id(p) for p in ps)
         rest = [p for p in ema.params if id(p) not in fused]
         st = C.c_void_p(torch.cuda.current_stream().cuda_stream)
```

Result: no change. 6393 images/s (median of 5 runs) (+0.2%).
